# cambrian-mllm/cambrian

Measured on NVIDIA H100. Metric: train_samples_per_sec, higher is better.
Workload: dtype bf16

## Files before the change

cambrian_b200/csrc/attention.cu:

```cuda
#include "common.cuh"
#include <cudaTypedefs.h>
#include <type_traits>

namespace cb {

int make_tmap_bf16_4d(CUtensorMap* out, const void* base, uint64_t d0, uint64_t d1, uint64_t d2, uint64_t d3,
                      uint64_t s1, uint64_t s2, uint64_t s3, uint32_t box_rows);

constexpr float LOG2E = 1.4426950408889634f;

struct AttnParams {
  bf16* o;
  long long o_bs, o_ss;
  float* lse;
  const uint8_t* kmask;
  int B, nh, nkv, Sq, Skv, hd, causal;
  float scale_log2;
};

template <int N>
__device__ __forceinline__ bool keys_all_valid(const uint8_t* km, int k0) {
  constexpr int PER = N / 32;
  static_assert(PER == 2 || PER == 4, "64- or 128-key tiles");
  const uint8_t* kp = km + k0 + PER * (threadIdx.x & 31);
  uint32_t w = 0;
  if (!(reinterpret_cast<uintptr_t>(kp) & (PER - 1))) {
    w = PER == 4 ? *reinterpret_cast<const uint32_t*>(kp) : *reinterpret_cast<const uint16_t*>(kp);
  } else {
#pragma unroll
    for (int i = 0; i < PER; ++i) w |= (uint32_t)kp[i] << (8 * i);
  }
  bool ok = true;
#pragma unroll
  for (int i = 0; i < PER; ++i) ok = ok && ((w >> (8 * i)) & 0xffu);
  return __all_sync(0xffffffffu, ok);
}

struct TileIdx {
  int t, h, b;
};
__device__ __forceinline__ TileIdx tile_index(int heads, int B) {
  const int hb = heads * B;
  const int rem = (int)blockIdx.x % hb;
  return {(int)blockIdx.x / hb, rem % heads, rem / heads};
}

template <int HDP>
struct FwdCfg {
  static constexpr int ATOMS = (HDP + 63) / 64;
  static constexpr int TILE = ATOMS * 16384;
  static constexpr int STAGES = 3;
  static constexpr int SMEM = TILE * (1 + 2 * STAGES) + 1024 + 256;
};

template <int HDP>
__global__ void __launch_bounds__(288, 1)
attn_fwd_kernel(const __grid_constant__ CUtensorMap tmQ, const __grid_constant__ CUtensorMap tmK,
                const __grid_constant__ CUtensorMap tmV, AttnParams p) {
  using Cfg = FwdCfg<HDP>;
  constexpr int STAGES = Cfg::STAGES;
  extern __shared__ uint8_t smem_raw[];
  const uint32_t base = (smem_u32(smem_raw) + 1023u) & ~1023u;
  const uint32_t sQ = base;
  const uint32_t sK = sQ + Cfg::TILE;
  const uint32_t sV = sK + STAGES * Cfg::TILE;
  const uint32_t bars = sV + STAGES * Cfg::TILE;
  const uint32_t q_full = bars;
  auto k_full = [&](int s) { return bars + 8u * (1 + s); };
  auto v_full = [&](int s) { return bars + 8u * (1 + STAGES + s); };
  auto kv_empty = [&](int s) { return bars + 8u * (1 + 2 * STAGES + s); };

  const int warp = threadIdx.x >> 5, lane = threadIdx.x & 31;
  const int q_tiles = (p.Sq + 127) / 128;
  const TileIdx ti = tile_index(p.nh, p.B);
  const int qt = q_tiles - 1 - ti.t;
  const int h = ti.h, b = ti.b;
  const int hk = h / (p.nh / p.nkv);
  const int q0 = qt * 128;
  const int kv_tiles_all = (p.Skv + 127) / 128;
  const int coff = p.Skv - p.Sq;
  int n_tiles = kv_tiles_all;
  if (p.causal) {
    const int last_key = q0 + 127 + coff;
    n_tiles = min(kv_tiles_all, last_key / 128 + 1);
    if (n_tiles < 1) n_tiles = 1;
  }

  if (warp == 8 && lane == 0) {
    tma_prefetch_desc(&tmQ);
    tma_prefetch_desc(&tmK);
    tma_prefetch_desc(&tmV);
    mbar_init(q_full, 1);
    for (int s = 0; s < STAGES; ++s) {
      mbar_init(k_full(s), 1);
      mbar_init(v_full(s), 1);
      mbar_init(kv_empty(s), 2);
    }
    mbar_fence_init();
  }
  __syncthreads();

  if (warp == 8) {
    if (lane == 0) {
      mbar_arrive_expect_tx(q_full, Cfg::TILE);
#pragma unroll
      for (int a = 0; a < Cfg::ATOMS; ++a) tma_load_4d(sQ + a * 16384, &tmQ, q_full, a * 64, h, q0, b);
      int st = 0;
      uint32_t ph = 0;
      for (int j = 0; j < n_tiles; ++j) {
        mbar_wait(kv_empty(st), ph ^ 1u);
        mbar_arrive_expect_tx(k_full(st), Cfg::TILE);
#pragma unroll
        for (int a = 0; a < Cfg::ATOMS; ++a)
          tma_load_4d(sK + st * Cfg::TILE + a * 16384, &tmK, k_full(st), a * 64, hk, j * 128, b);
        mbar_arrive_expect_tx(v_full(st), Cfg::TILE);
#pragma unroll
        for (int a = 0; a < Cfg::ATOMS; ++a)
          tma_load_4d(sV + st * Cfg::TILE + a * 16384, &tmV, v_full(st), a * 64, hk, j * 128, b);
        if (++st == STAGES) { st = 0; ph ^= 1u; }
      }
    }
    return;
  }

  const int wg = warp >> 2;
  const bool wg_leader = (threadIdx.x & 127) == 0;
  const int rloc = wg * 64 + (warp & 3) * 16 + (lane >> 2);
  const int cq = 2 * (lane & 3);
  const uint8_t* km = p.kmask ? p.kmask + (size_t)b * p.Skv : nullptr;
  float o[HDP / 2];
#pragma unroll
  for (int i = 0; i < HDP / 2; ++i) o[i] = 0.f;
  float m_run[2] = {-INFINITY, -INFINITY}, l_run[2] = {0.f, 0.f};
  mbar_wait(q_full, 0);
  int st = 0;
  uint32_t ph = 0;
  for (int j = 0; j < n_tiles; ++j) {
    const int k0 = j * 128;
    float s[64];
    mbar_wait(k_full(st), ph);
    const uint32_t kb = sK + st * Cfg::TILE;
    wgmma_fence();
#pragma unroll
    for (int kk = 0; kk < HDP / 16; ++kk) {
      const uint32_t off = (kk >> 2) * 16384 + (kk & 3) * 32;
      WgmmaSS<128, 0, 0>::mma(s, make_smem_desc_sw128(sQ + wg * 8192 + off, 0, 1024),
                              make_smem_desc_sw128(kb + off, 0, 1024), kk ? 1u : 0u);
    }
    wgmma_commit();
    bool full_tile = k0 + 128 <= p.Skv && (!p.causal || k0 + 127 <= q0 + wg * 64 + coff);
    if (full_tile && km) full_tile = keys_all_valid<128>(km, k0);
    wgmma_wait<0>();
    reg_fence(s);
    float mx[2] = {-INFINITY, -INFINITY};
#pragma unroll
    for (int jj = 0; jj < 16; ++jj) {
#pragma unroll
      for (int e = 0; e < 4; ++e) {
        float v = s[4 * jj + e] * p.scale_log2;
        if (!full_tile) {
          const int key = k0 + 8 * jj + cq + (e & 1);
          const int qi = q0 + rloc + 8 * (e >> 1);
          const bool ok = key < p.Skv && (!p.causal || key <= qi + coff) && (!km || km[key]);
          v = ok ? v : -INFINITY;
        }
        s[4 * jj + e] = v;
        mx[e >> 1] = fmaxf(mx[e >> 1], v);
      }
    }
    float corr[2], mref[2];
#pragma unroll
    for (int r = 0; r < 2; ++r) {
      mx[r] = fmaxf(mx[r], __shfl_xor_sync(0xffffffffu, mx[r], 1));
      mx[r] = fmaxf(mx[r], __shfl_xor_sync(0xffffffffu, mx[r], 2));
      const float m_new = fmaxf(m_run[r], mx[r]);
      mref[r] = m_new == -INFINITY ? 0.f : m_new;
      corr[r] = fast_exp2(m_run[r] - mref[r]);
      m_run[r] = m_new;
      l_run[r] *= corr[r];
    }
#pragma unroll
    for (int jj = 0; jj < HDP / 8; ++jj) {
#pragma unroll
      for (int e = 0; e < 4; ++e) o[4 * jj + e] *= corr[e >> 1];
    }
    uint32_t pa[8][4];
#pragma unroll
    for (int jj = 0; jj < 16; ++jj) {
      float pv[4];
#pragma unroll
      for (int e = 0; e < 4; ++e) {
        pv[e] = fast_exp2(s[4 * jj + e] - mref[e >> 1]);
        l_run[e >> 1] += pv[e];
      }
      pa[jj >> 1][(jj & 1) * 2 + 0] = pack_bf16x2(pv[0], pv[1]);
      pa[jj >> 1][(jj & 1) * 2 + 1] = pack_bf16x2(pv[2], pv[3]);
    }
    mbar_wait(v_full(st), ph);
    const uint32_t vb = sV + st * Cfg::TILE;
    reg_fence(o);
    wgmma_fence();
#pragma unroll
    for (int kk = 0; kk < 8; ++kk)
      WgmmaRS<HDP, 1>::mma(o, pa[kk], make_smem_desc_sw128(vb + kk * 2048, 16384, 1024), 1u);
    wgmma_commit();
    wgmma_wait<0>();
    reg_fence(o);
    if (wg_leader) mbar_arrive(kv_empty(st));
    if (++st == STAGES) { st = 0; ph ^= 1u; }
  }
#pragma unroll
  for (int r = 0; r < 2; ++r) {
    float l = l_run[r];
    l += __shfl_xor_sync(0xffffffffu, l, 1);
    l += __shfl_xor_sync(0xffffffffu, l, 2);
    const int qi = q0 + rloc + 8 * r;
    if (qi >= p.Sq) continue;
    const float inv = l > 0.f ? 1.f / l : 0.f;
    bf16* op = p.o + (long long)b * p.o_bs + (long long)qi * p.o_ss + (long long)h * p.hd;
#pragma unroll
    for (int jj = 0; jj < HDP / 8; ++jj) {
      const int d = 8 * jj + cq;
      if (d < p.hd)
        *reinterpret_cast<__nv_bfloat162*>(op + d) = __floats2bfloat162_rn(o[4 * jj + 2 * r] * inv, o[4 * jj + 2 * r + 1] * inv);
    }
    if (p.lse && (lane & 3) == 0)
      p.lse[((long long)b * p.nh + h) * p.Sq + qi] = l > 0.f ? m_run[r] + log2f(l) : INFINITY;
  }
}

__global__ void attn_delta_kernel(const bf16* __restrict__ o, const bf16* __restrict__ d_o, float* __restrict__ delta,
                                  int B, int S, int nh, int hd, long long o_bs, long long o_ss, long long do_bs,
                                  long long do_ss) {
  const int lph = hd >> 3;
  const int hpw = 32 / lph;
  const long long w = (blockIdx.x * (long long)blockDim.x + threadIdx.x) >> 5;
  const int lane = threadIdx.x & 31;
  const long long total = (long long)B * S * nh;
  const long long idx = w * hpw + lane / lph;
  const int sub = lane % lph;
  float acc = 0.f;
  if (idx < total) {
    const int h = (int)(idx % nh);
    const long long t = idx / nh;
    const int s = (int)(t % S);
    const int b = (int)(t / S);
    const bf16* op = o + b * o_bs + s * o_ss + (long long)h * hd + sub * 8;
    const bf16* gp = d_o + b * do_bs + s * do_ss + (long long)h * hd + sub * 8;
    float a[8], g[8];
    unpack8(ldg_nc(op), a);
    unpack8(ldg_nc(gp), g);
#pragma unroll
    for (int e = 0; e < 8; ++e) acc += a[e] * g[e];
  }
  for (int off = lph >> 1; off > 0; off >>= 1) acc += __shfl_xor_sync(0xffffffffu, acc, off);
  if (idx < total && sub == 0) {
    const int h = (int)(idx % nh);
    const long long t = idx / nh;
    delta[((long long)(t / S) * nh + h) * S + (t % S)] = acc;
  }
}

struct AttnBwdParams {
  bf16* dq;
  bf16* dk;
  bf16* dv;
  long long dq_bs, dq_ss, dk_bs, dk_ss, dv_bs, dv_ss;
  const float* lse;
  const float* delta;
  const uint8_t* kmask;
  int B, nh, nkv, Sq, Skv, hd, causal;
  float scale_log2, scale;
};

template <int HDP>
struct BwdCfg {
  static constexpr int ATOMS = HDP / 64;
  static constexpr int KTILE = ATOMS * 16384;
  static constexpr int QTILE = ATOMS * 8192;
  static constexpr int STAGES = 4;
  static constexpr int SMEM = 2 * KTILE + 2 * STAGES * QTILE + STAGES * 512 + 1024 + 256;
};

template <int HDP>
__global__ void __launch_bounds__(384, 1)
attn_bwd_kernel(const __grid_constant__ CUtensorMap tmQ, const __grid_constant__ CUtensorMap tmK,
                const __grid_constant__ CUtensorMap tmV, const __grid_constant__ CUtensorMap tmdO, AttnBwdParams p) {
  using Cfg = BwdCfg<HDP>;
  constexpr int STAGES = Cfg::STAGES;
  extern __shared__ uint8_t smem_raw[];
  const uint32_t base = (smem_u32(smem_raw) + 1023u) & ~1023u;
  const uint32_t sK = base;
  const uint32_t sV = sK + Cfg::KTILE;
  const uint32_t sQ = sV + Cfg::KTILE;
  const uint32_t sdO = sQ + STAGES * Cfg::QTILE;
  const uint32_t sLD = sdO + STAGES * Cfg::QTILE;
  const uint32_t bars = sLD + STAGES * 512;
  const uint32_t kv_full = bars;
  auto qd_full = [&](int s) { return bars + 8u * (1 + s); };
  auto qd_empty = [&](int s) { return bars + 8u * (1 + STAGES + s); };
  float* ld_stage = reinterpret_cast<float*>(smem_raw + (sLD - smem_u32(smem_raw)));

  const int warp = threadIdx.x >> 5, lane = threadIdx.x & 31;
  const TileIdx ti = tile_index(p.nkv, p.B);
  const int jt = ti.t, g = ti.h, b = ti.b;
  const int G = p.nh / p.nkv;
  const int k0 = jt * 128;
  const int q_tiles = (p.Sq + 63) / 64;
  const int coff = p.Skv - p.Sq;
  int i_begin = 0;
  if (p.causal) {
    const int first_q = k0 - coff;
    i_begin = first_q > 0 ? first_q / 64 : 0;
  }
  const int n_i = q_tiles > i_begin ? q_tiles - i_begin : 0;
  const int n_iter = n_i * G;

  if (warp == 8 && lane == 0) {
    tma_prefetch_desc(&tmQ);
    tma_prefetch_desc(&tmK);
    tma_prefetch_desc(&tmV);
    tma_prefetch_desc(&tmdO);
    mbar_init(kv_full, 1);
    for (int s = 0; s < STAGES; ++s) {
      mbar_init(qd_full(s), 1 + 32);
      mbar_init(qd_empty(s), 8);
    }
    mbar_fence_init();
  }
  __syncthreads();

  if (warp >= 8) {
    setmaxnreg_dec<24>();
    if (warp > 8) return;
    if (lane == 0) {
      mbar_arrive_expect_tx(kv_full, 2 * Cfg::KTILE);
#pragma unroll
      for (int a = 0; a < Cfg::ATOMS; ++a) {
        tma_load_4d(sK + a * 16384, &tmK, kv_full, a * 64, g, k0, b);
        tma_load_4d(sV + a * 16384, &tmV, kv_full, a * 64, g, k0, b);
      }
    }
    int st = 0;
    uint32_t ph = 0;
    for (int it = 0; it < n_iter; ++it) {
      const int h = g * G + it / n_i;
      const int qi0 = (i_begin + it % n_i) * 64;
      mbar_wait(qd_empty(st), ph ^ 1u);
      if (lane == 0) {
        mbar_arrive_expect_tx(qd_full(st), 2 * Cfg::QTILE);
#pragma unroll
        for (int a = 0; a < Cfg::ATOMS; ++a) {
          tma_load_4d(sQ + st * Cfg::QTILE + a * 8192, &tmQ, qd_full(st), a * 64, h, qi0, b);
          tma_load_4d(sdO + st * Cfg::QTILE + a * 8192, &tmdO, qd_full(st), a * 64, h, qi0, b);
        }
      }
      const float* lse = p.lse + ((long long)b * p.nh + h) * p.Sq;
      const float* dlt = p.delta + ((long long)b * p.nh + h) * p.Sq;
      float* ld = ld_stage + st * 128;
#pragma unroll
      for (int i = lane; i < 64; i += 32) {
        const int qi = qi0 + i;
        ld[i] = qi < p.Sq ? __ldg(lse + qi) : 0.f;
        ld[64 + i] = qi < p.Sq ? __ldg(dlt + qi) : 0.f;
      }
      mbar_arrive(qd_full(st));
      if (++st == STAGES) { st = 0; ph ^= 1u; }
    }
    return;
  }

  setmaxnreg_inc<240>();
  const int wg = warp >> 2;
  const int kr = wg * 64 + (warp & 3) * 16 + (lane >> 2);
  const int cq = 2 * (lane & 3);
  const int wk0 = k0 + wg * 64 + (warp & 3) * 16;
  bool key_ok[2];
#pragma unroll
  for (int r = 0; r < 2; ++r) {
    const int kidx = k0 + kr + 8 * r;
    key_ok[r] = kidx < p.Skv && (!p.kmask || p.kmask[(size_t)b * p.Skv + kidx]);
  }
  const bool warp_keys_ok = __all_sync(0xffffffffu, key_ok[0] && key_ok[1]);
  float dv[HDP / 2], dk[HDP / 2];
#pragma unroll
  for (int i = 0; i < HDP / 2; ++i) dv[i] = dk[i] = 0.f;
  mbar_wait(kv_full, 0);
  int st = 0;
  uint32_t ph = 0;
  for (int it = 0; it < n_iter; ++it) {
    const int qi0 = (i_begin + it % n_i) * 64;
    const uint32_t qb = sQ + st * Cfg::QTILE, dob = sdO + st * Cfg::QTILE;
    mbar_wait(qd_full(st), ph);
    float sT[32], dpT[32];
    wgmma_fence();
#pragma unroll
    for (int kk = 0; kk < HDP / 16; ++kk) {
      const uint32_t koff = (kk >> 2) * 16384 + (kk & 3) * 32, qoff = (kk >> 2) * 8192 + (kk & 3) * 32;
      WgmmaSS<64, 0, 0>::mma(sT, make_smem_desc_sw128(sK + wg * 8192 + koff, 0, 1024),
                             make_smem_desc_sw128(qb + qoff, 0, 1024), kk ? 1u : 0u);
    }
#pragma unroll
    for (int kk = 0; kk < HDP / 16; ++kk) {
      const uint32_t koff = (kk >> 2) * 16384 + (kk & 3) * 32, qoff = (kk >> 2) * 8192 + (kk & 3) * 32;
      WgmmaSS<64, 0, 0>::mma(dpT, make_smem_desc_sw128(sV + wg * 8192 + koff, 0, 1024),
                             make_smem_desc_sw128(dob + qoff, 0, 1024), kk ? 1u : 0u);
    }
    wgmma_commit();
    const bool full = warp_keys_ok && qi0 + 64 <= p.Sq && (!p.causal || wk0 + 15 <= qi0 + coff);
    const float* ld = ld_stage + st * 128;
    wgmma_wait<0>();
    reg_fence(sT);
    reg_fence(dpT);
    uint32_t pa[4][4], da[4][4];
    auto grads = [&](auto full_tile) {
#pragma unroll
      for (int jj = 0; jj < 8; ++jj) {
        float pv[4], dsv[4];
#pragma unroll
        for (int c = 0; c < 2; ++c) {
          const int qc = 8 * jj + cq + c;
          const float L = ld[qc], D = ld[64 + qc];
#pragma unroll
          for (int r = 0; r < 2; ++r) {
            const int e = 2 * r + c;
            bool vis = true;
            if (!decltype(full_tile)::value)
              vis = qi0 + qc < p.Sq && key_ok[r] && (!p.causal || k0 + kr + 8 * r <= qi0 + qc + coff);
            const float pe = vis ? fast_exp2(fmaf(sT[4 * jj + e], p.scale_log2, -L)) : 0.f;
            pv[e] = pe;
            dsv[e] = pe * (dpT[4 * jj + e] - D);
          }
        }
        pa[jj >> 1][(jj & 1) * 2 + 0] = pack_bf16x2(pv[0], pv[1]);
        pa[jj >> 1][(jj & 1) * 2 + 1] = pack_bf16x2(pv[2], pv[3]);
        da[jj >> 1][(jj & 1) * 2 + 0] = pack_bf16x2(dsv[0], dsv[1]);
        da[jj >> 1][(jj & 1) * 2 + 1] = pack_bf16x2(dsv[2], dsv[3]);
      }
    };
    if (full)
      grads(std::true_type());
    else
      grads(std::false_type());
    reg_fence(dv);
    reg_fence(dk);
    wgmma_fence();
#pragma unroll
    for (int kk = 0; kk < 4; ++kk) {
      WgmmaRS<HDP, 1>::mma(dv, pa[kk], make_smem_desc_sw128(dob + kk * 2048, 8192, 1024), 1u);
      WgmmaRS<HDP, 1>::mma(dk, da[kk], make_smem_desc_sw128(qb + kk * 2048, 8192, 1024), 1u);
    }
    wgmma_commit();
    wgmma_wait<0>();
    reg_fence(dv);
    reg_fence(dk);
    if (lane == 0) mbar_arrive(qd_empty(st));
    if (++st == STAGES) { st = 0; ph ^= 1u; }
  }
#pragma unroll
  for (int r = 0; r < 2; ++r) {
    const int kidx = k0 + kr + 8 * r;
    if (kidx >= p.Skv) continue;
    bf16* dkp = p.dk + (long long)b * p.dk_bs + (long long)kidx * p.dk_ss + (long long)g * p.hd;
    bf16* dvp = p.dv + (long long)b * p.dv_bs + (long long)kidx * p.dv_ss + (long long)g * p.hd;
#pragma unroll
    for (int jj = 0; jj < HDP / 8; ++jj) {
      const int d = 8 * jj + cq;
      *reinterpret_cast<__nv_bfloat162*>(dkp + d) =
          __floats2bfloat162_rn(dk[4 * jj + 2 * r] * p.scale, dk[4 * jj + 2 * r + 1] * p.scale);
      *reinterpret_cast<__nv_bfloat162*>(dvp + d) = __floats2bfloat162_rn(dv[4 * jj + 2 * r], dv[4 * jj + 2 * r + 1]);
    }
  }
}

template <int HDP>
struct DqCfg {
  static constexpr int ATOMS = HDP / 64;
  static constexpr int QTILE = ATOMS * 16384;
  static constexpr int KTILE = ATOMS * 8192;
  static constexpr int STAGES = 4;
  static constexpr int SMEM = 2 * QTILE + 2 * STAGES * KTILE + 1024 + 256;
};

template <int HDP>
__global__ void __launch_bounds__(288, 1)
attn_bwd_dq_kernel(const __grid_constant__ CUtensorMap tmQ, const __grid_constant__ CUtensorMap tmK,
                   const __grid_constant__ CUtensorMap tmV, const __grid_constant__ CUtensorMap tmdO, AttnBwdParams p) {
  using Cfg = DqCfg<HDP>;
  constexpr int STAGES = Cfg::STAGES;
  extern __shared__ uint8_t smem_raw[];
  const uint32_t base = (smem_u32(smem_raw) + 1023u) & ~1023u;
  const uint32_t sQ = base;
  const uint32_t sdO = sQ + Cfg::QTILE;
  const uint32_t sK = sdO + Cfg::QTILE;
  const uint32_t sV = sK + STAGES * Cfg::KTILE;
  const uint32_t bars = sV + STAGES * Cfg::KTILE;
  const uint32_t q_full = bars;
  auto kv_full = [&](int s) { return bars + 8u * (1 + s); };
  auto kv_empty = [&](int s) { return bars + 8u * (1 + STAGES + s); };

  const int warp = threadIdx.x >> 5, lane = threadIdx.x & 31;
  const int q_tiles = (p.Sq + 127) / 128;
  const TileIdx ti = tile_index(p.nh, p.B);
  const int qt = q_tiles - 1 - ti.t;
  const int h = ti.h, b = ti.b;
  const int hk = h / (p.nh / p.nkv);
  const int q0 = qt * 128;
  const int coff = p.Skv - p.Sq;
  const int kv_tiles_all = (p.Skv + 63) / 64;
  int n_tiles = kv_tiles_all;
  if (p.causal) n_tiles = max(1, min(kv_tiles_all, (q0 + 127 + coff) / 64 + 1));

  if (warp == 8 && lane == 0) {
    tma_prefetch_desc(&tmQ);
    tma_prefetch_desc(&tmK);
    tma_prefetch_desc(&tmV);
    tma_prefetch_desc(&tmdO);
    mbar_init(q_full, 1);
    for (int s = 0; s < STAGES; ++s) {
      mbar_init(kv_full(s), 1);
      mbar_init(kv_empty(s), 2);
    }
    mbar_fence_init();
  }
  __syncthreads();

  if (warp == 8) {
    if (lane == 0) {
      mbar_arrive_expect_tx(q_full, 2 * Cfg::QTILE);
#pragma unroll
      for (int a = 0; a < Cfg::ATOMS; ++a) {
        tma_load_4d(sQ + a * 16384, &tmQ, q_full, a * 64, h, q0, b);
        tma_load_4d(sdO + a * 16384, &tmdO, q_full, a * 64, h, q0, b);
      }
      int st = 0;
      uint32_t ph = 0;
      for (int j = 0; j < n_tiles; ++j) {
        mbar_wait(kv_empty(st), ph ^ 1u);
        mbar_arrive_expect_tx(kv_full(st), 2 * Cfg::KTILE);
#pragma unroll
        for (int a = 0; a < Cfg::ATOMS; ++a) {
          tma_load_4d(sK + st * Cfg::KTILE + a * 8192, &tmK, kv_full(st), a * 64, hk, j * 64, b);
          tma_load_4d(sV + st * Cfg::KTILE + a * 8192, &tmV, kv_full(st), a * 64, hk, j * 64, b);
        }
        if (++st == STAGES) { st = 0; ph ^= 1u; }
      }
    }
    return;
  }

  const int wg = warp >> 2;
  const bool wg_leader = (threadIdx.x & 127) == 0;
  const int rloc = wg * 64 + (warp & 3) * 16 + (lane >> 2);
  const int cq = 2 * (lane & 3);
  const int wq0 = q0 + wg * 64 + (warp & 3) * 16;
  const uint8_t* km = p.kmask ? p.kmask + (size_t)b * p.Skv : nullptr;
  const float* lse = p.lse + ((long long)b * p.nh + h) * p.Sq;
  const float* dlt = p.delta + ((long long)b * p.nh + h) * p.Sq;
  int qi[2];
  float L[2], D[2];
#pragma unroll
  for (int r = 0; r < 2; ++r) {
    qi[r] = q0 + rloc + 8 * r;
    L[r] = qi[r] < p.Sq ? __ldg(lse + qi[r]) : 0.f;
    D[r] = qi[r] < p.Sq ? __ldg(dlt + qi[r]) : 0.f;
  }
  float dq[HDP / 2];
#pragma unroll
  for (int i = 0; i < HDP / 2; ++i) dq[i] = 0.f;
  mbar_wait(q_full, 0);
  int st = 0;
  uint32_t ph = 0;
  for (int j = 0; j < n_tiles; ++j) {
    const int k0 = j * 64;
    mbar_wait(kv_full(st), ph);
    const uint32_t kb = sK + st * Cfg::KTILE, vb = sV + st * Cfg::KTILE;
    float s[32], dp[32];
    wgmma_fence();
#pragma unroll
    for (int kk = 0; kk < HDP / 16; ++kk) {
      const uint32_t qoff = wg * 8192 + (kk >> 2) * 16384 + (kk & 3) * 32, koff = (kk >> 2) * 8192 + (kk & 3) * 32;
      WgmmaSS<64, 0, 0>::mma(s, make_smem_desc_sw128(sQ + qoff, 0, 1024), make_smem_desc_sw128(kb + koff, 0, 1024),
                             kk ? 1u : 0u);
    }
#pragma unroll
    for (int kk = 0; kk < HDP / 16; ++kk) {
      const uint32_t qoff = wg * 8192 + (kk >> 2) * 16384 + (kk & 3) * 32, koff = (kk >> 2) * 8192 + (kk & 3) * 32;
      WgmmaSS<64, 0, 0>::mma(dp, make_smem_desc_sw128(sdO + qoff, 0, 1024), make_smem_desc_sw128(vb + koff, 0, 1024),
                             kk ? 1u : 0u);
    }
    wgmma_commit();
    bool full = k0 + 64 <= p.Skv && wq0 + 16 <= p.Sq && (!p.causal || k0 + 63 <= wq0 + coff);
    if (full && km) full = keys_all_valid<64>(km, k0);
    wgmma_wait<0>();
    reg_fence(s);
    reg_fence(dp);
    uint32_t da[4][4];
    auto grads = [&](auto full_tile) {
#pragma unroll
      for (int jj = 0; jj < 8; ++jj) {
        float dsv[4];
#pragma unroll
        for (int e = 0; e < 4; ++e) {
          const int r = e >> 1, key = k0 + 8 * jj + cq + (e & 1);
          bool vis = true;
          if (!decltype(full_tile)::value)
            vis = qi[r] < p.Sq && key < p.Skv && (!p.causal || key <= qi[r] + coff) && (!km || km[key]);
          const float pe = vis ? fast_exp2(fmaf(s[4 * jj + e], p.scale_log2, -L[r])) : 0.f;
          dsv[e] = pe * (dp[4 * jj + e] - D[r]);
        }
        da[jj >> 1][(jj & 1) * 2 + 0] = pack_bf16x2(dsv[0], dsv[1]);
        da[jj >> 1][(jj & 1) * 2 + 1] = pack_bf16x2(dsv[2], dsv[3]);
      }
    };
    if (full)
      grads(std::true_type());
    else
      grads(std::false_type());
    reg_fence(dq);
    wgmma_fence();
#pragma unroll
    for (int kk = 0; kk < 4; ++kk)
      WgmmaRS<HDP, 1>::mma(dq, da[kk], make_smem_desc_sw128(kb + kk * 2048, 8192, 1024), 1u);
    wgmma_commit();
    wgmma_wait<0>();
    reg_fence(dq);
    if (wg_leader) mbar_arrive(kv_empty(st));
    if (++st == STAGES) { st = 0; ph ^= 1u; }
  }
#pragma unroll
  for (int r = 0; r < 2; ++r) {
    if (qi[r] >= p.Sq) continue;
    bf16* dqp = p.dq + (long long)b * p.dq_bs + (long long)qi[r] * p.dq_ss + (long long)h * p.hd;
#pragma unroll
    for (int jj = 0; jj < HDP / 8; ++jj)
      *reinterpret_cast<__nv_bfloat162*>(dqp + 8 * jj + cq) =
          __floats2bfloat162_rn(dq[4 * jj + 2 * r] * p.scale, dq[4 * jj + 2 * r + 1] * p.scale);
  }
}

static PFN_cuTensorMapEncodeTiled_v12000 encode_fn() {
  static PFN_cuTensorMapEncodeTiled_v12000 fn = nullptr;
  if (!fn) {
    void* ptr = nullptr;
    cudaDriverEntryPointQueryResult q;
    if (cudaGetDriverEntryPoint("cuTensorMapEncodeTiled", &ptr, cudaEnableDefault, &q) == cudaSuccess &&
        q == cudaDriverEntryPointSuccess)
      fn = reinterpret_cast<PFN_cuTensorMapEncodeTiled_v12000>(ptr);
  }
  return fn;
}

int make_tmap_bf16_4d(CUtensorMap* out, const void* base, uint64_t d0, uint64_t d1, uint64_t d2, uint64_t d3,
                      uint64_t s1, uint64_t s2, uint64_t s3, uint32_t box_rows) {
  auto fn = encode_fn();
  if (!fn) return set_error(CB_ERR_CUDA, "cuTensorMapEncodeTiled entry point not available");
  if ((reinterpret_cast<uintptr_t>(base) & 15u) || (s1 % 8) || (s2 % 8) || (d3 > 1 && (s3 % 8)))
    return set_error(CB_ERR_INVALID, "attention: operands must be 16-byte aligned with strides %% 8 == 0");
  cuuint64_t dims[4] = {d0, d1, d2, d3};
  cuuint64_t strides[3] = {s1 * 2, s2 * 2, (d3 > 1 ? s3 : s2 * d2) * 2};
  cuuint32_t box[4] = {64, 1, box_rows, 1};
  cuuint32_t estr[4] = {1, 1, 1, 1};
  CUresult r = fn(out, CU_TENSOR_MAP_DATA_TYPE_BFLOAT16, 4, const_cast<void*>(base), dims, strides, box, estr,
                  CU_TENSOR_MAP_INTERLEAVE_NONE, CU_TENSOR_MAP_SWIZZLE_128B, CU_TENSOR_MAP_L2_PROMOTION_L2_256B,
                  CU_TENSOR_MAP_FLOAT_OOB_FILL_NONE);
  if (r == CUDA_ERROR_INVALID_CONTEXT) {
    cudaFree(0);
    r = fn(out, CU_TENSOR_MAP_DATA_TYPE_BFLOAT16, 4, const_cast<void*>(base), dims, strides, box, estr,
           CU_TENSOR_MAP_INTERLEAVE_NONE, CU_TENSOR_MAP_SWIZZLE_128B, CU_TENSOR_MAP_L2_PROMOTION_L2_256B,
           CU_TENSOR_MAP_FLOAT_OOB_FILL_NONE);
  }
  if (r != CUDA_SUCCESS) return set_error(CB_ERR_CUDA, "cuTensorMapEncodeTiled(4d) failed (%d)", (int)r);
  return CB_OK;
}

static int hd_padded(int hd) { return (hd + 15) / 16 * 16; }

template <int HDP>
static int launch_fwd(const CUtensorMap& tq, const CUtensorMap& tk, const CUtensorMap& tv, const AttnParams& p,
                      cudaStream_t st) {
  using Cfg = FwdCfg<HDP>;
  auto kern = attn_fwd_kernel<HDP>;
  static bool attr = false;
  if (!attr) {
    cudaError_t e = cudaFuncSetAttribute(kern, cudaFuncAttributeMaxDynamicSharedMemorySize, Cfg::SMEM);
    if (e != cudaSuccess) return set_error(CB_ERR_CUDA, "attn fwd smem attr: %s", cudaGetErrorString(e));
    attr = true;
  }
  kern<<<(p.Sq + 127) / 128 * p.nh * p.B, 288, Cfg::SMEM, st>>>(tq, tk, tv, p);
  CB_CUDA_LAUNCH_CHECK("attn_fwd");
  return CB_OK;
}

int attn_fwd_launch(const void* q, const void* k, const void* v, void* o, float* lse, const void* kmask, int B,
                    int nh, int nkv, int Sq, int Skv, int hd, long long q_bs, long long q_ss, long long k_bs,
                    long long k_ss, long long v_bs, long long v_ss, long long o_bs, long long o_ss, float scale,
                    int causal, cudaStream_t st) {
  CB_CHECK_ARG(B > 0 && nh > 0 && nkv > 0 && Sq > 0 && Skv > 0, "attention: empty problem");
  CB_CHECK_ARG(nh % nkv == 0, "attention: nh=%d not a multiple of nkv=%d", nh, nkv);
  CB_CHECK_ARG(hd % 8 == 0 && hd <= 128, "attention: head_dim=%d must be a multiple of 8 and <= 128", hd);
  CB_CHECK_ARG(o_ss % 8 == 0 && o_bs % 8 == 0 && !(reinterpret_cast<uintptr_t>(o) & 15u),
               "attention: output must be 16-byte aligned with strides %% 8 == 0");
  CUtensorMap tq, tk, tv;
  int rc;
  if ((rc = make_tmap_bf16_4d(&tq, q, hd, nh, Sq, B, hd, q_ss, q_bs, 128))) return rc;
  if ((rc = make_tmap_bf16_4d(&tk, k, hd, nkv, Skv, B, hd, k_ss, k_bs, 128))) return rc;
  if ((rc = make_tmap_bf16_4d(&tv, v, hd, nkv, Skv, B, hd, v_ss, v_bs, 128))) return rc;
  AttnParams p;
  p.o = (bf16*)o; p.o_bs = o_bs; p.o_ss = o_ss; p.lse = lse; p.kmask = (const uint8_t*)kmask;
  p.B = B; p.nh = nh; p.nkv = nkv; p.Sq = Sq; p.Skv = Skv; p.hd = hd; p.causal = causal;
  p.scale_log2 = scale * LOG2E;
  const int hdp = hd_padded(hd);
  if (hdp <= 64) return launch_fwd<64>(tq, tk, tv, p, st);
  if (hdp <= 80) return launch_fwd<80>(tq, tk, tv, p, st);
  if (hdp <= 96) return launch_fwd<96>(tq, tk, tv, p, st);
  return launch_fwd<128>(tq, tk, tv, p, st);
}

template <int HDP>
static int launch_bwd(const CUtensorMap& tq, const CUtensorMap& tk, const CUtensorMap& tv, const CUtensorMap& tdo,
                      const AttnBwdParams& p, cudaStream_t st) {
  using Cfg = BwdCfg<HDP>;
  auto kern = attn_bwd_kernel<HDP>;
  static bool attr = false;
  if (!attr) {
    cudaError_t e = cudaFuncSetAttribute(kern, cudaFuncAttributeMaxDynamicSharedMemorySize, Cfg::SMEM);
    if (e != cudaSuccess) return set_error(CB_ERR_CUDA, "attn bwd smem attr: %s", cudaGetErrorString(e));
    attr = true;
  }
  kern<<<(p.Skv + 127) / 128 * p.nkv * p.B, 384, Cfg::SMEM, st>>>(tq, tk, tv, tdo, p);
  CB_CUDA_LAUNCH_CHECK("attn_bwd");
  return CB_OK;
}

template <int HDP>
static int launch_bwd_dq(const CUtensorMap& tq, const CUtensorMap& tk, const CUtensorMap& tv, const CUtensorMap& tdo,
                         const AttnBwdParams& p, cudaStream_t st) {
  using Cfg = DqCfg<HDP>;
  auto kern = attn_bwd_dq_kernel<HDP>;
  static bool attr = false;
  if (!attr) {
    cudaError_t e = cudaFuncSetAttribute(kern, cudaFuncAttributeMaxDynamicSharedMemorySize, Cfg::SMEM);
    if (e != cudaSuccess) return set_error(CB_ERR_CUDA, "attn bwd dq smem attr: %s", cudaGetErrorString(e));
    attr = true;
  }
  kern<<<(p.Sq + 127) / 128 * p.nh * p.B, 288, Cfg::SMEM, st>>>(tq, tk, tv, tdo, p);
  CB_CUDA_LAUNCH_CHECK("attn_bwd_dq");
  return CB_OK;
}

int attn_bwd_launch(const void* q, const void* k, const void* v, const void* o, const void* d_o, const float* lse,
                    float* delta, void* dq, void* dk, void* dv, const void* kmask, int B, int nh, int nkv,
                    int Sq, int Skv, int hd, long long q_bs, long long q_ss, long long k_bs, long long k_ss,
                    long long v_bs, long long v_ss, long long o_bs, long long o_ss, long long do_bs, long long do_ss,
                    long long dq_bs, long long dq_ss, long long dk_bs, long long dk_ss, long long dv_bs,
                    long long dv_ss, float scale, int causal, cudaStream_t st) {
  CB_CHECK_ARG(B > 0 && nh > 0 && nkv > 0 && Sq > 0 && Skv > 0, "attention bwd: empty problem");
  CB_CHECK_ARG(nh % nkv == 0, "attention bwd: nh=%d not a multiple of nkv=%d", nh, nkv);
  CB_CHECK_ARG(hd == 64 || hd == 128, "attention bwd: head_dim=%d unsupported (64 or 128)", hd);
  CB_CHECK_ARG(lse && delta && dq && dk && dv, "attention bwd: lse / delta / dq / dk / dv buffers are required");
  CB_CHECK_ARG(!(reinterpret_cast<uintptr_t>(dq) & 3u) && dq_bs % 2 == 0 && dq_ss % 2 == 0,
               "attention bwd: dq must be 4-byte aligned with even strides");
  {
    const long long warps = ((long long)B * Sq * nh + (256 / hd) - 1) / (256 / hd);
    attn_delta_kernel<<<(unsigned)((warps * 32 + 255) / 256), 256, 0, st>>>((const bf16*)o, (const bf16*)d_o, delta, B,
                                                                           Sq, nh, hd, o_bs, o_ss, do_bs, do_ss);
    CB_CUDA_LAUNCH_CHECK("attn_delta");
  }
  CUtensorMap tq, tk, tv, tdo;
  int rc;
  if ((rc = make_tmap_bf16_4d(&tq, q, hd, nh, Sq, B, hd, q_ss, q_bs, 64))) return rc;
  if ((rc = make_tmap_bf16_4d(&tk, k, hd, nkv, Skv, B, hd, k_ss, k_bs, 128))) return rc;
  if ((rc = make_tmap_bf16_4d(&tv, v, hd, nkv, Skv, B, hd, v_ss, v_bs, 128))) return rc;
  if ((rc = make_tmap_bf16_4d(&tdo, d_o, hd, nh, Sq, B, hd, do_ss, do_bs, 64))) return rc;
  AttnBwdParams p;
  p.dq = (bf16*)dq; p.dk = (bf16*)dk; p.dv = (bf16*)dv;
  p.dq_bs = dq_bs; p.dq_ss = dq_ss; p.dk_bs = dk_bs; p.dk_ss = dk_ss; p.dv_bs = dv_bs; p.dv_ss = dv_ss;
  p.lse = lse; p.delta = delta; p.kmask = (const uint8_t*)kmask;
  p.B = B; p.nh = nh; p.nkv = nkv; p.Sq = Sq; p.Skv = Skv; p.hd = hd; p.causal = causal;
  p.scale_log2 = scale * LOG2E; p.scale = scale;
  CUtensorMap tq128, tk64, tv64, tdo128;
  if ((rc = make_tmap_bf16_4d(&tq128, q, hd, nh, Sq, B, hd, q_ss, q_bs, 128))) return rc;
  if ((rc = make_tmap_bf16_4d(&tk64, k, hd, nkv, Skv, B, hd, k_ss, k_bs, 64))) return rc;
  if ((rc = make_tmap_bf16_4d(&tv64, v, hd, nkv, Skv, B, hd, v_ss, v_bs, 64))) return rc;
  if ((rc = make_tmap_bf16_4d(&tdo128, d_o, hd, nh, Sq, B, hd, do_ss, do_bs, 128))) return rc;
  if (hd == 64) {
    if ((rc = launch_bwd<64>(tq, tk, tv, tdo, p, st))) return rc;
    return launch_bwd_dq<64>(tq128, tk64, tv64, tdo128, p, st);
  }
  if ((rc = launch_bwd<128>(tq, tk, tv, tdo, p, st))) return rc;
  return launch_bwd_dq<128>(tq128, tk64, tv64, tdo128, p, st);
}

}
```

cambrian_b200/csrc/common.cuh:

```cuda
#pragma once
#include <cuda_runtime.h>
#include <cuda_bf16.h>
#include <cuda.h>
#include <stdint.h>
#include "wgmma.cuh"

namespace cb {

typedef __nv_bfloat16 bf16;

int set_error(int code, const char* fmt, ...);
#define CB_OK 0
#define CB_ERR_INVALID 1
#define CB_ERR_CUDA 2
#define CB_ERR_UNSUPPORTED 3

#define CB_CHECK_ARG(cond, ...)                                         \
  do {                                                                  \
    if (!(cond)) return cb::set_error(CB_ERR_INVALID, __VA_ARGS__);     \
  } while (0)

void count_launch();
#define CB_CUDA_LAUNCH_CHECK(name)                                                    \
  do {                                                                                \
    cb::count_launch();                                                               \
    cudaError_t _e = cudaGetLastError();                                              \
    if (_e != cudaSuccess)                                                            \
      return cb::set_error(CB_ERR_CUDA, "%s: %s", name, cudaGetErrorString(_e));      \
  } while (0)

int device_sm_count();

__device__ __forceinline__ float warp_sum(float v) {
#pragma unroll
  for (int o = 16; o > 0; o >>= 1) v += __shfl_xor_sync(0xffffffffu, v, o);
  return v;
}
__device__ __forceinline__ float warp_max(float v) {
#pragma unroll
  for (int o = 16; o > 0; o >>= 1) v = fmaxf(v, __shfl_xor_sync(0xffffffffu, v, o));
  return v;
}

__device__ __forceinline__ float fast_exp2(float x) {
  float y;
  asm("ex2.approx.ftz.f32 %0, %1;" : "=f"(y) : "f"(x));
  return y;
}
__device__ __forceinline__ float fast_rcp(float x) {
  float y;
  asm("rcp.approx.ftz.f32 %0, %1;" : "=f"(y) : "f"(x));
  return y;
}
__device__ __forceinline__ float erf_fast(float x) {
  const float ax = fabsf(x);
  const float t = __fdividef(1.0f, fmaf(0.3275911f, ax, 1.0f));
  float y = fmaf(t, 1.061405429f, -1.453152027f);
  y = fmaf(t, y, 1.421413741f);
  y = fmaf(t, y, -0.284496736f);
  y = fmaf(t, y, 0.254829592f);
  const float r = fmaf(-t * y, __expf(-ax * ax), 1.0f);
  return copysignf(r, x);
}
__device__ __forceinline__ float gelu_erf(float x) {
  const float ax = fabsf(x);
  const float t = fast_rcp(fmaf(0.3275911f * 0.70710678118654752440f, ax, 1.0f));
  float y = fmaf(t, 1.061405429f, -1.453152027f);
  y = fmaf(t, y, 1.421413741f);
  y = fmaf(t, y, -0.284496736f);
  y = fmaf(t, y, 0.254829592f);
  const float e = fast_exp2(x * x * -0.72134752044448170368f);
  const float r = fmaf(-(y * t), e, 1.0f);
  const float hx = 0.5f * x;
  return fmaf(fabsf(hx), r, hx);
}
__device__ __forceinline__ float gelu_erf_grad(float x) {
  const float cdf = 0.5f * (1.0f + erf_fast(x * 0.70710678118654752440f));
  const float pdf = 0.39894228040143267794f * __expf(-0.5f * x * x);
  return cdf + x * pdf;
}
__device__ __forceinline__ float gelu_tanh(float x) {
  const float u = 0.7978845608028654f * (x + 0.044715f * x * x * x);
  return 0.5f * x * (1.0f + tanhf(u));
}
__device__ __forceinline__ float gelu_tanh_fast(float x) {
  const float u = 0.7978845608028654f * (x + 0.044715f * x * x * x);
  const float t = 1.0f - 2.0f * fast_rcp(1.0f + fast_exp2(2.0f * 1.44269504088896340736f * u));
  return 0.5f * x * (1.0f + t);
}
__device__ __forceinline__ float quick_gelu(float x) { return x * fast_rcp(1.0f + fast_exp2(-1.702f * 1.44269504088896340736f * x)); }
__device__ __forceinline__ float silu(float x) { return x * fast_rcp(1.0f + fast_exp2(-1.44269504088896340736f * x)); }

struct alignas(16) bf16x8 {
  __nv_bfloat162 v[4];
};
__device__ __forceinline__ void unpack8(const uint4& u, float* f) {
  const __nv_bfloat162* p = reinterpret_cast<const __nv_bfloat162*>(&u);
#pragma unroll
  for (int i = 0; i < 4; ++i) {
    float2 t = __bfloat1622float2(p[i]);
    f[2 * i] = t.x;
    f[2 * i + 1] = t.y;
  }
}
__device__ __forceinline__ uint4 pack8(const float* f) {
  uint4 u;
  __nv_bfloat162* p = reinterpret_cast<__nv_bfloat162*>(&u);
#pragma unroll
  for (int i = 0; i < 4; ++i) p[i] = __floats2bfloat162_rn(f[2 * i], f[2 * i + 1]);
  return u;
}
__device__ __forceinline__ uint4 ldg_nc(const void* p) {
  uint4 r;
  asm volatile("ld.global.nc.L1::no_allocate.v4.u32 {%0,%1,%2,%3}, [%4];"
               : "=r"(r.x), "=r"(r.y), "=r"(r.z), "=r"(r.w)
               : "l"(p));
  return r;
}

__device__ __forceinline__ uint32_t smem_u32(const void* p) {
  return static_cast<uint32_t>(__cvta_generic_to_shared(p));
}
__device__ __forceinline__ void mbar_init(uint32_t bar, uint32_t count) {
  asm volatile("mbarrier.init.shared::cta.b64 [%0], %1;" ::"r"(bar), "r"(count));
}
__device__ __forceinline__ void mbar_fence_init() {
  asm volatile("fence.mbarrier_init.release.cluster;" ::: "memory");
}
__device__ __forceinline__ void mbar_arrive_expect_tx(uint32_t bar, uint32_t bytes) {
  asm volatile("mbarrier.arrive.expect_tx.shared::cta.b64 _, [%0], %1;" ::"r"(bar), "r"(bytes)
               : "memory");
}
__device__ __forceinline__ void mbar_arrive(uint32_t bar) {
  asm volatile("mbarrier.arrive.shared::cta.b64 _, [%0];" ::"r"(bar) : "memory");
}
__device__ __forceinline__ void mbar_wait(uint32_t bar, uint32_t parity) {
  uint32_t done;
  do {
    asm volatile(
        "{\n"
        ".reg .pred p;\n"
        "mbarrier.try_wait.parity.shared::cta.b64 p, [%1], %2;\n"
        "selp.u32 %0, 1, 0, p;\n"
        "}\n"
        : "=r"(done)
        : "r"(bar), "r"(parity)
        : "memory");
  } while (!done);
}
__device__ __forceinline__ void st_shared_b32(uint32_t addr, uint32_t v) {
  asm volatile("st.shared.b32 [%0], %1;" ::"r"(addr), "r"(v) : "memory");
}
__device__ __forceinline__ void fence_proxy_async_smem() {
  asm volatile("fence.proxy.async.shared::cta;" ::: "memory");
}

__device__ __forceinline__ void tma_prefetch_desc(const CUtensorMap* m) {
  asm volatile("prefetch.tensormap [%0];" ::"l"(m) : "memory");
}
__device__ __forceinline__ void tma_load_3d(uint32_t smem_dst, const CUtensorMap* m, uint32_t bar,
                                            int c0, int c1, int c2) {
  asm volatile(
      "cp.async.bulk.tensor.3d.shared::cluster.global.mbarrier::complete_tx::bytes "
      "[%0], [%1, {%3, %4, %5}], [%2];"
      :
      : "r"(smem_dst), "l"(m), "r"(bar), "r"(c0), "r"(c1), "r"(c2)
      : "memory");
}
__device__ __forceinline__ void tma_load_4d(uint32_t smem_dst, const CUtensorMap* m, uint32_t bar,
                                            int c0, int c1, int c2, int c3) {
  asm volatile(
      "cp.async.bulk.tensor.4d.shared::cluster.global.mbarrier::complete_tx::bytes "
      "[%0], [%1, {%3, %4, %5, %6}], [%2];"
      :
      : "r"(smem_dst), "l"(m), "r"(bar), "r"(c0), "r"(c1), "r"(c2), "r"(c3)
      : "memory");
}
__device__ __forceinline__ void tma_store_3d(const CUtensorMap* m, uint32_t smem_src, int c0, int c1, int c2) {
  asm volatile("cp.async.bulk.tensor.3d.global.shared::cta.bulk_group [%0, {%2, %3, %4}], [%1];"
               :
               : "l"(m), "r"(smem_src), "r"(c0), "r"(c1), "r"(c2)
               : "memory");
}
__device__ __forceinline__ void bulk_commit() { asm volatile("cp.async.bulk.commit_group;" ::: "memory"); }
template <int N>
__device__ __forceinline__ void bulk_wait_read() {
  asm volatile("cp.async.bulk.wait_group.read %0;" ::"n"(N) : "memory");
}
template <int N>
__device__ __forceinline__ void bulk_wait() {
  asm volatile("cp.async.bulk.wait_group %0;" ::"n"(N) : "memory");
}
template <int N>
__device__ __forceinline__ void setmaxnreg_dec() { asm volatile("setmaxnreg.dec.sync.aligned.u32 %0;" ::"n"(N)); }
template <int N>
__device__ __forceinline__ void setmaxnreg_inc() { asm volatile("setmaxnreg.inc.sync.aligned.u32 %0;" ::"n"(N)); }
__device__ __forceinline__ void named_bar_sync(int id, int threads) {
  asm volatile("bar.sync %0, %1;" ::"r"(id), "r"(threads) : "memory");
}

__device__ __forceinline__ void wgmma_fence() { asm volatile("wgmma.fence.sync.aligned;" ::: "memory"); }
__device__ __forceinline__ void wgmma_commit() { asm volatile("wgmma.commit_group.sync.aligned;" ::: "memory"); }
template <int N>
__device__ __forceinline__ void wgmma_wait() {
  asm volatile("wgmma.wait_group.sync.aligned %0;" ::"n"(N) : "memory");
}
template <int R>
__device__ __forceinline__ void reg_fence(float (&d)[R]) {
#pragma unroll
  for (int i = 0; i < R; ++i) asm volatile("" : "+f"(d[i])::"memory");
}

__device__ __forceinline__ uint64_t make_smem_desc_sw128(uint32_t saddr, uint32_t lbo_bytes,
                                                         uint32_t sbo_bytes) {
  uint64_t d = 0;
  d |= static_cast<uint64_t>((saddr & 0x3FFFFu) >> 4);
  d |= static_cast<uint64_t>((lbo_bytes >> 4) & 0x3FFFu) << 16;
  d |= static_cast<uint64_t>((sbo_bytes >> 4) & 0x3FFFu) << 32;
  d |= static_cast<uint64_t>(1) << 62;
  return d;
}

__device__ __forceinline__ uint32_t pack_bf16x2(float lo, float hi) {
  __nv_bfloat162 t = __floats2bfloat162_rn(lo, hi);
  return *reinterpret_cast<uint32_t*>(&t);
}

}
```

Before: 7.913.

## Make attention fwd/bwd-dq kernels persistent with pingpong warpgroups and TMA output stores

Converts the attention forward and backward-dQ kernels into persistent kernels that loop over work tiles in serpentine order, launching at most one CTA per SM. A double-buffered Q stage is added, and K and V get separate empty barriers. The two consumer warpgroups are interleaved with named barriers (pingpong), and the next S GEMM is overlapped with the current PV GEMM. Register budgets are reallocated with setmaxnreg, and the output is written through a TMA store from shared memory when alignment allows. This targets launch and tail overhead and aims to hide softmax latency behind tensor-core work, at the cost of much more complex synchronisation and fewer pipeline stages.

```diff
diff --git a/cambrian_b200/csrc/attention.cu b/cambrian_b200/csrc/attention.cu
--- a/cambrian_b200/csrc/attention.cu
+++ b/cambrian_b200/csrc/attention.cu
@@ -1,5 +1,6 @@
 #include "common.cuh"
 #include <cudaTypedefs.h>
+#include <algorithm>
 #include <type_traits>
 
 namespace cb {
@@ -16,6 +17,7 @@
   const uint8_t* kmask;
   int B, nh, nkv, Sq, Skv, hd, causal;
   float scale_log2;
+  int tma_store;
 };
 
 template <int N>
@@ -39,194 +41,298 @@
 struct TileIdx {
   int t, h, b;
 };
-__device__ __forceinline__ TileIdx tile_index(int heads, int B) {
+__device__ __forceinline__ TileIdx tile_index(int w, int heads, int B) {
   const int hb = heads * B;
-  const int rem = (int)blockIdx.x % hb;
-  return {(int)blockIdx.x / hb, rem % heads, rem / heads};
+  const int rem = w % hb;
+  return {w / hb, rem % heads, rem / heads};
+}
+__device__ __forceinline__ int work_tile(int k) {
+  const int G = gridDim.x, c = blockIdx.x;
+  return k * G + ((k & 1) ? G - 1 - c : c);
 }
 
 template <int HDP>
 struct FwdCfg {
   static constexpr int ATOMS = (HDP + 63) / 64;
   static constexpr int TILE = ATOMS * 16384;
-  static constexpr int STAGES = 3;
-  static constexpr int SMEM = TILE * (1 + 2 * STAGES) + 1024 + 256;
+  static constexpr int SMEM = 6 * TILE + 1024 + 256;
 };
 
 template <int HDP>
-__global__ void __launch_bounds__(288, 1)
+__global__ void __launch_bounds__(384, 1)
 attn_fwd_kernel(const __grid_constant__ CUtensorMap tmQ, const __grid_constant__ CUtensorMap tmK,
-                const __grid_constant__ CUtensorMap tmV, AttnParams p) {
+                const __grid_constant__ CUtensorMap tmV, const __grid_constant__ CUtensorMap tmO, AttnParams p) {
   using Cfg = FwdCfg<HDP>;
-  constexpr int STAGES = Cfg::STAGES;
   extern __shared__ uint8_t smem_raw[];
   const uint32_t base = (smem_u32(smem_raw) + 1023u) & ~1023u;
   const uint32_t sQ = base;
-  const uint32_t sK = sQ + Cfg::TILE;
-  const uint32_t sV = sK + STAGES * Cfg::TILE;
-  const uint32_t bars = sV + STAGES * Cfg::TILE;
-  const uint32_t q_full = bars;
-  auto k_full = [&](int s) { return bars + 8u * (1 + s); };
-  auto v_full = [&](int s) { return bars + 8u * (1 + STAGES + s); };
-  auto kv_empty = [&](int s) { return bars + 8u * (1 + 2 * STAGES + s); };
+  const uint32_t sK = sQ + 2 * Cfg::TILE;
+  const uint32_t sV = sK + 2 * Cfg::TILE;
+  const uint32_t bars = sV + 2 * Cfg::TILE;
+  auto q_full = [&](int s) { return bars + 8u * s; };
+  auto q_empty = [&](int s) { return bars + 8u * (2 + s); };
+  auto k_full = [&](int s) { return bars + 8u * (4 + s); };
+  auto k_empty = [&](int s) { return bars + 8u * (6 + s); };
+  auto v_full = [&](int s) { return bars + 8u * (8 + s); };
+  auto v_empty = [&](int s) { return bars + 8u * (10 + s); };
 
   const int warp = threadIdx.x >> 5, lane = threadIdx.x & 31;
   const int q_tiles = (p.Sq + 127) / 128;
-  const TileIdx ti = tile_index(p.nh, p.B);
-  const int qt = q_tiles - 1 - ti.t;
-  const int h = ti.h, b = ti.b;
-  const int hk = h / (p.nh / p.nkv);
-  const int q0 = qt * 128;
+  const int work = q_tiles * p.nh * p.B;
   const int kv_tiles_all = (p.Skv + 127) / 128;
   const int coff = p.Skv - p.Sq;
-  int n_tiles = kv_tiles_all;
-  if (p.causal) {
-    const int last_key = q0 + 127 + coff;
-    n_tiles = min(kv_tiles_all, last_key / 128 + 1);
-    if (n_tiles < 1) n_tiles = 1;
-  }
+  auto key_tiles = [&](int q0) {
+    return p.causal ? max(1, min(kv_tiles_all, (q0 + 127 + coff) / 128 + 1)) : kv_tiles_all;
+  };
 
   if (warp == 8 && lane == 0) {
     tma_prefetch_desc(&tmQ);
     tma_prefetch_desc(&tmK);
     tma_prefetch_desc(&tmV);
-    mbar_init(q_full, 1);
-    for (int s = 0; s < STAGES; ++s) {
+    for (int s = 0; s < 2; ++s) {
+      mbar_init(q_full(s), 1);
+      mbar_init(q_empty(s), 2);
       mbar_init(k_full(s), 1);
+      mbar_init(k_empty(s), 2);
       mbar_init(v_full(s), 1);
-      mbar_init(kv_empty(s), 2);
+      mbar_init(v_empty(s), 2);
     }
     mbar_fence_init();
   }
   __syncthreads();
 
-  if (warp == 8) {
-    if (lane == 0) {
-      mbar_arrive_expect_tx(q_full, Cfg::TILE);
-#pragma unroll
-      for (int a = 0; a < Cfg::ATOMS; ++a) tma_load_4d(sQ + a * 16384, &tmQ, q_full, a * 64, h, q0, b);
-      int st = 0;
-      uint32_t ph = 0;
-      for (int j = 0; j < n_tiles; ++j) {
-        mbar_wait(kv_empty(st), ph ^ 1u);
-        mbar_arrive_expect_tx(k_full(st), Cfg::TILE);
+  if (warp >= 8) {
+    setmaxnreg_dec<24>();
+    if (warp == 8 && lane == 0) {
+      int qs = 0, st = 0;
+      uint32_t qph = 0, ph = 0;
+      for (int k = 0, w; (w = work_tile(k)) < work; ++k) {
+        const TileIdx ti = tile_index(w, p.nh, p.B);
+        const int q0 = (q_tiles - 1 - ti.t) * 128;
+        const int hk = ti.h / (p.nh / p.nkv);
+        mbar_wait(q_empty(qs), qph ^ 1u);
+        mbar_arrive_expect_tx(q_full(qs), Cfg::TILE);
 #pragma unroll
         for (int a = 0; a < Cfg::ATOMS; ++a)
-          tma_load_4d(sK + st * Cfg::TILE + a * 16384, &tmK, k_full(st), a * 64, hk, j * 128, b);
-        mbar_arrive_expect_tx(v_full(st), Cfg::TILE);
-#pragma unroll
-        for (int a = 0; a < Cfg::ATOMS; ++a)
-          tma_load_4d(sV + st * Cfg::TILE + a * 16384, &tmV, v_full(st), a * 64, hk, j * 128, b);
-        if (++st == STAGES) { st = 0; ph ^= 1u; }
+          tma_load_4d(sQ + qs * Cfg::TILE + a * 16384, &tmQ, q_full(qs), a * 64, ti.h, q0, ti.b);
+        if (++qs == 2) { qs = 0; qph ^= 1u; }
+        const int n_tiles = key_tiles(q0);
+        for (int j = 0; j < n_tiles; ++j) {
+          mbar_wait(k_empty(st), ph ^ 1u);
+          mbar_arrive_expect_tx(k_full(st), Cfg::TILE);
+#pragma unroll
+          for (int a = 0; a < Cfg::ATOMS; ++a)
+            tma_load_4d(sK + st * Cfg::TILE + a * 16384, &tmK, k_full(st), a * 64, hk, j * 128, ti.b);
+          mbar_wait(v_empty(st), ph ^ 1u);
+          mbar_arrive_expect_tx(v_full(st), Cfg::TILE);
+#pragma unroll
+          for (int a = 0; a < Cfg::ATOMS; ++a)
+            tma_load_4d(sV + st * Cfg::TILE + a * 16384, &tmV, v_full(st), a * 64, hk, j * 128, ti.b);
+          if (++st == 2) { st = 0; ph ^= 1u; }
+        }
       }
     }
     return;
   }
 
+  setmaxnreg_inc<240>();
   const int wg = warp >> 2;
   const bool wg_leader = (threadIdx.x & 127) == 0;
-  const int rloc = wg * 64 + (warp & 3) * 16 + (lane >> 2);
+  const int srow = (warp & 3) * 16 + (lane >> 2);
+  const int rloc = wg * 64 + srow;
   const int cq = 2 * (lane & 3);
-  const uint8_t* km = p.kmask ? p.kmask + (size_t)b * p.Skv : nullptr;
-  float o[HDP / 2];
-#pragma unroll
-  for (int i = 0; i < HDP / 2; ++i) o[i] = 0.f;
-  float m_run[2] = {-INFINITY, -INFINITY}, l_run[2] = {0.f, 0.f};
-  mbar_wait(q_full, 0);
-  int st = 0;
-  uint32_t ph = 0;
-  for (int j = 0; j < n_tiles; ++j) {
-    const int k0 = j * 128;
-    float s[64];
-    mbar_wait(k_full(st), ph);
-    const uint32_t kb = sK + st * Cfg::TILE;
+  const int bar_mine = 1 + wg, bar_other = 2 - wg;
+  if (wg == 1) named_bar_arrive(1, 256);
+  if (wg_leader && p.tma_store) tma_prefetch_desc(&tmO);
+
+  int qs = 0, kst = 0, vst = 0;
+  uint32_t qph = 0, kph = 0, vph = 0;
+  int q_release = -1;
+  for (int k = 0, w; (w = work_tile(k)) < work; ++k) {
+    const TileIdx ti = tile_index(w, p.nh, p.B);
+    const int q0 = (q_tiles - 1 - ti.t) * 128;
+    const int h = ti.h, b = ti.b;
+    const int n_tiles = key_tiles(q0);
+    const uint8_t* km = p.kmask ? p.kmask + (size_t)b * p.Skv : nullptr;
+    const uint32_t qb = sQ + qs * Cfg::TILE + wg * 8192;
+    float o[HDP / 2], s[64];
+    uint32_t pa[8][4];
+#pragma unroll
+    for (int i = 0; i < HDP / 2; ++i) o[i] = 0.f;
+    float m_run[2] = {-INFINITY, -INFINITY}, l_run[2] = {0.f, 0.f}, corr[2];
+
+    auto issue_s = [&]() {
+      const uint32_t kb = sK + kst * Cfg::TILE;
+#pragma unroll
+      for (int kk = 0; kk < HDP / 16; ++kk) {
+        const uint32_t off = (kk >> 2) * 16384 + (kk & 3) * 32;
+        WgmmaSS<128, 0, 0>::mma(s, make_smem_desc_sw128(qb + off, 0, 1024), make_smem_desc_sw128(kb + off, 0, 1024),
+                                kk ? 1u : 0u);
+      }
+      wgmma_commit();
+    };
+    auto tile_full = [&](int k0) {
+      bool full = k0 + 128 <= p.Skv && (!p.causal || k0 + 127 <= q0 + wg * 64 + coff);
+      if (full && km) full = keys_all_valid<128>(km, k0);
+      return full;
+    };
+    auto softmax = [&](int k0, bool full_tile) {
+      float mx[2] = {-INFINITY, -INFINITY};
+#pragma unroll
+      for (int jj = 0; jj < 16; ++jj) {
+#pragma unroll
+        for (int e = 0; e < 4; ++e) {
+          float v = s[4 * jj + e] * p.scale_log2;
+          if (!full_tile) {
+            const int key = k0 + 8 * jj + cq + (e & 1);
+            const int qi = q0 + rloc + 8 * (e >> 1);
+            const bool ok = key < p.Skv && (!p.causal || key <= qi + coff) && (!km || km[key]);
+            v = ok ? v : -INFINITY;
+          }
+          s[4 * jj + e] = v;
+          mx[e >> 1] = fmaxf(mx[e >> 1], v);
+        }
+      }
+      float mref[2];
+#pragma unroll
+      for (int r = 0; r < 2; ++r) {
+        mx[r] = fmaxf(mx[r], __shfl_xor_sync(0xffffffffu, mx[r], 1));
+        mx[r] = fmaxf(mx[r], __shfl_xor_sync(0xffffffffu, mx[r], 2));
+        const float m_new = fmaxf(m_run[r], mx[r]);
+        mref[r] = m_new == -INFINITY ? 0.f : m_new;
+        corr[r] = fast_exp2(m_run[r] - mref[r]);
+        m_run[r] = m_new;
+        l_run[r] *= corr[r];
+      }
+#pragma unroll
+      for (int jj = 0; jj < 16; ++jj) {
+#pragma unroll
+        for (int e = 0; e < 4; ++e) {
+          s[4 * jj + e] = fast_exp2(s[4 * jj + e] - mref[e >> 1]);
+          l_run[e >> 1] += s[4 * jj + e];
+        }
+      }
+    };
+    auto rescale_pack = [&]() {
+#pragma unroll
+      for (int jj = 0; jj < HDP / 8; ++jj) {
+#pragma unroll
+        for (int e = 0; e < 4; ++e) o[4 * jj + e] *= corr[e >> 1];
+      }
+#pragma unroll
+      for (int jj = 0; jj < 16; ++jj) {
+        pa[jj >> 1][(jj & 1) * 2 + 0] = pack_bf16x2(s[4 * jj + 0], s[4 * jj + 1]);
+        pa[jj >> 1][(jj & 1) * 2 + 1] = pack_bf16x2(s[4 * jj + 2], s[4 * jj + 3]);
+      }
+    };
+
+    mbar_wait(q_full(qs), qph);
+    mbar_wait(k_full(kst), kph);
+    named_bar_sync(bar_mine, 256);
     wgmma_fence();
-#pragma unroll
-    for (int kk = 0; kk < HDP / 16; ++kk) {
-      const uint32_t off = (kk >> 2) * 16384 + (kk & 3) * 32;
-      WgmmaSS<128, 0, 0>::mma(s, make_smem_desc_sw128(sQ + wg * 8192 + off, 0, 1024),
-                              make_smem_desc_sw128(kb + off, 0, 1024), kk ? 1u : 0u);
-    }
-    wgmma_commit();
-    bool full_tile = k0 + 128 <= p.Skv && (!p.causal || k0 + 127 <= q0 + wg * 64 + coff);
-    if (full_tile && km) full_tile = keys_all_valid<128>(km, k0);
-    wgmma_wait<0>();
-    reg_fence(s);
-    float mx[2] = {-INFINITY, -INFINITY};
-#pragma unroll
-    for (int jj = 0; jj < 16; ++jj) {
-#pragma unroll
-      for (int e = 0; e < 4; ++e) {
-        float v = s[4 * jj + e] * p.scale_log2;
-        if (!full_tile) {
-          const int key = k0 + 8 * jj + cq + (e & 1);
-          const int qi = q0 + rloc + 8 * (e >> 1);
-          const bool ok = key < p.Skv && (!p.causal || key <= qi + coff) && (!km || km[key]);
-          v = ok ? v : -INFINITY;
-        }
-        s[4 * jj + e] = v;
-        mx[e >> 1] = fmaxf(mx[e >> 1], v);
-      }
-    }
-    float corr[2], mref[2];
-#pragma unroll
-    for (int r = 0; r < 2; ++r) {
-      mx[r] = fmaxf(mx[r], __shfl_xor_sync(0xffffffffu, mx[r], 1));
-      mx[r] = fmaxf(mx[r], __shfl_xor_sync(0xffffffffu, mx[r], 2));
-      const float m_new = fmaxf(m_run[r], mx[r]);
-      mref[r] = m_new == -INFINITY ? 0.f : m_new;
-      corr[r] = fast_exp2(m_run[r] - mref[r]);
-      m_run[r] = m_new;
-      l_run[r] *= corr[r];
-    }
-#pragma unroll
-    for (int jj = 0; jj < HDP / 8; ++jj) {
-#pragma unroll
-      for (int e = 0; e < 4; ++e) o[4 * jj + e] *= corr[e >> 1];
-    }
-    uint32_t pa[8][4];
-#pragma unroll
-    for (int jj = 0; jj < 16; ++jj) {
-      float pv[4];
-#pragma unroll
-      for (int e = 0; e < 4; ++e) {
-        pv[e] = fast_exp2(s[4 * jj + e] - mref[e >> 1]);
-        l_run[e >> 1] += pv[e];
-      }
-      pa[jj >> 1][(jj & 1) * 2 + 0] = pack_bf16x2(pv[0], pv[1]);
-      pa[jj >> 1][(jj & 1) * 2 + 1] = pack_bf16x2(pv[2], pv[3]);
-    }
-    mbar_wait(v_full(st), ph);
-    const uint32_t vb = sV + st * Cfg::TILE;
+    issue_s();
+    named_bar_arrive(bar_other, 256);
+    if (q_release >= 0 && wg_leader) {
+      if (p.tma_store) bulk_wait_read<0>();
+      mbar_arrive(q_empty(q_release));
+    }
+    {
+      const bool full = tile_full(0);
+      wgmma_wait<0>();
+      reg_fence(s);
+      if (wg_leader) mbar_arrive(k_empty(kst));
+      if (++kst == 2) { kst = 0; kph ^= 1u; }
+      softmax(0, full);
+      rescale_pack();
+    }
+    auto issue_pv = [&]() {
+      const uint32_t vb = sV + vst * Cfg::TILE;
+#pragma unroll
+      for (int kk = 0; kk < 8; ++kk)
+        WgmmaRS<HDP, 1>::mma(o, pa[kk], make_smem_desc_sw128(vb + kk * 2048, 16384, 1024), 1u);
+      wgmma_commit();
+    };
+    auto release_v = [&]() {
+      if (wg_leader) mbar_arrive(v_empty(vst));
+      if (++vst == 2) { vst = 0; vph ^= 1u; }
+    };
+    for (int j = 0; j + 1 < n_tiles; ++j) {
+      mbar_wait(k_full(kst), kph);
+      mbar_wait(v_full(vst), vph);
+      named_bar_sync(bar_mine, 256);
+      reg_fence(o);
+      wgmma_fence();
+      issue_s();
+      issue_pv();
+      named_bar_arrive(bar_other, 256);
+      const int k1 = (j + 1) * 128;
+      const bool full = tile_full(k1);
+      wgmma_wait<1>();
+      reg_fence(s);
+      if (wg_leader) mbar_arrive(k_empty(kst));
+      if (++kst == 2) { kst = 0; kph ^= 1u; }
+      softmax(k1, full);
+      wgmma_wait<0>();
+      reg_fence(o);
+      release_v();
+      rescale_pack();
+    }
+    mbar_wait(v_full(vst), vph);
+    named_bar_sync(bar_mine, 256);
     reg_fence(o);
     wgmma_fence();
-#pragma unroll
-    for (int kk = 0; kk < 8; ++kk)
-      WgmmaRS<HDP, 1>::mma(o, pa[kk], make_smem_desc_sw128(vb + kk * 2048, 16384, 1024), 1u);
-    wgmma_commit();
+    issue_pv();
+    named_bar_arrive(bar_other, 256);
     wgmma_wait<0>();
     reg_fence(o);
-    if (wg_leader) mbar_arrive(kv_empty(st));
-    if (++st == STAGES) { st = 0; ph ^= 1u; }
-  }
-#pragma unroll
-  for (int r = 0; r < 2; ++r) {
-    float l = l_run[r];
-    l += __shfl_xor_sync(0xffffffffu, l, 1);
-    l += __shfl_xor_sync(0xffffffffu, l, 2);
-    const int qi = q0 + rloc + 8 * r;
-    if (qi >= p.Sq) continue;
-    const float inv = l > 0.f ? 1.f / l : 0.f;
-    bf16* op = p.o + (long long)b * p.o_bs + (long long)qi * p.o_ss + (long long)h * p.hd;
-#pragma unroll
-    for (int jj = 0; jj < HDP / 8; ++jj) {
-      const int d = 8 * jj + cq;
-      if (d < p.hd)
-        *reinterpret_cast<__nv_bfloat162*>(op + d) = __floats2bfloat162_rn(o[4 * jj + 2 * r] * inv, o[4 * jj + 2 * r + 1] * inv);
-    }
-    if (p.lse && (lane & 3) == 0)
-      p.lse[((long long)b * p.nh + h) * p.Sq + qi] = l > 0.f ? m_run[r] + log2f(l) : INFINITY;
-  }
+    release_v();
+    float inv[2];
+#pragma unroll
+    for (int r = 0; r < 2; ++r) {
+      float l = l_run[r];
+      l += __shfl_xor_sync(0xffffffffu, l, 1);
+      l += __shfl_xor_sync(0xffffffffu, l, 2);
+      inv[r] = l > 0.f ? 1.f / l : 0.f;
+      const int qi = q0 + rloc + 8 * r;
+      if (p.lse && (lane & 3) == 0 && qi < p.Sq)
+        p.lse[((long long)b * p.nh + h) * p.Sq + qi] = l > 0.f ? m_run[r] + log2f(l) : INFINITY;
+    }
+    if (p.tma_store) {
+#pragma unroll
+      for (int r = 0; r < 2; ++r) {
+        const int row = srow + 8 * r;
+#pragma unroll
+        for (int jj = 0; jj < HDP / 8; ++jj)
+          st_shared_b32(qb + (jj >> 3) * 16384 + row * 128 + (((jj & 7) ^ (row & 7)) << 4) + 2 * cq,
+                        pack_bf16x2(o[4 * jj + 2 * r] * inv[r], o[4 * jj + 2 * r + 1] * inv[r]));
+      }
+      fence_proxy_async_smem();
+      named_bar_sync(3 + wg, 128);
+      if (wg_leader) {
+#pragma unroll
+        for (int a = 0; a < Cfg::ATOMS; ++a) tma_store_4d(&tmO, qb + a * 16384, a * 64, h, q0 + wg * 64, b);
+        bulk_commit();
+      }
+    } else {
+#pragma unroll
+      for (int r = 0; r < 2; ++r) {
+        const int qi = q0 + rloc + 8 * r;
+        if (qi >= p.Sq) continue;
+        bf16* op = p.o + (long long)b * p.o_bs + (long long)qi * p.o_ss + (long long)h * p.hd;
+#pragma unroll
+        for (int jj = 0; jj < HDP / 8; ++jj) {
+          const int d = 8 * jj + cq;
+          if (d < p.hd)
+            *reinterpret_cast<__nv_bfloat162*>(op + d) =
+                __floats2bfloat162_rn(o[4 * jj + 2 * r] * inv[r], o[4 * jj + 2 * r + 1] * inv[r]);
+        }
+      }
+    }
+    q_release = qs;
+    if (++qs == 2) { qs = 0; qph ^= 1u; }
+  }
+  if (wg == 0) named_bar_sync(1, 256);
+  if (wg_leader && p.tma_store) bulk_wait<0>();
 }
 
 __global__ void attn_delta_kernel(const bf16* __restrict__ o, const bf16* __restrict__ d_o, float* __restrict__ delta,
@@ -302,7 +408,7 @@
   float* ld_stage = reinterpret_cast<float*>(smem_raw + (sLD - smem_u32(smem_raw)));
 
   const int warp = threadIdx.x >> 5, lane = threadIdx.x & 31;
-  const TileIdx ti = tile_index(p.nkv, p.B);
+  const TileIdx ti = tile_index(blockIdx.x, p.nkv, p.B);
   const int jt = ti.t, g = ti.h, b = ti.b;
   const int G = p.nh / p.nkv;
   const int k0 = jt * 128;
@@ -478,12 +584,12 @@
   static constexpr int ATOMS = HDP / 64;
   static constexpr int QTILE = ATOMS * 16384;
   static constexpr int KTILE = ATOMS * 8192;
-  static constexpr int STAGES = 4;
-  static constexpr int SMEM = 2 * QTILE + 2 * STAGES * KTILE + 1024 + 256;
+  static constexpr int STAGES = 3;
+  static constexpr int SMEM = 4 * QTILE + 2 * STAGES * KTILE + 1024 + 256;
 };
 
 template <int HDP>
-__global__ void __launch_bounds__(288, 1)
+__global__ void __launch_bounds__(384, 1)
 attn_bwd_dq_kernel(const __grid_constant__ CUtensorMap tmQ, const __grid_constant__ CUtensorMap tmK,
                    const __grid_constant__ CUtensorMap tmV, const __grid_constant__ CUtensorMap tmdO, AttnBwdParams p) {
   using Cfg = DqCfg<HDP>;
@@ -491,32 +597,33 @@
   extern __shared__ uint8_t smem_raw[];
   const uint32_t base = (smem_u32(smem_raw) + 1023u) & ~1023u;
   const uint32_t sQ = base;
-  const uint32_t sdO = sQ + Cfg::QTILE;
-  const uint32_t sK = sdO + Cfg::QTILE;
+  const uint32_t sdO = sQ + 2 * Cfg::QTILE;
+  const uint32_t sK = sdO + 2 * Cfg::QTILE;
   const uint32_t sV = sK + STAGES * Cfg::KTILE;
   const uint32_t bars = sV + STAGES * Cfg::KTILE;
-  const uint32_t q_full = bars;
-  auto kv_full = [&](int s) { return bars + 8u * (1 + s); };
-  auto kv_empty = [&](int s) { return bars + 8u * (1 + STAGES + s); };
+  auto q_full = [&](int s) { return bars + 8u * s; };
+  auto q_empty = [&](int s) { return bars + 8u * (2 + s); };
+  auto kv_full = [&](int s) { return bars + 8u * (4 + s); };
+  auto kv_empty = [&](int s) { return bars + 8u * (4 + STAGES + s); };
 
   const int warp = threadIdx.x >> 5, lane = threadIdx.x & 31;
   const int q_tiles = (p.Sq + 127) / 128;
-  const TileIdx ti = tile_index(p.nh, p.B);
-  const int qt = q_tiles - 1 - ti.t;
-  const int h = ti.h, b = ti.b;
-  const int hk = h / (p.nh / p.nkv);
-  const int q0 = qt * 128;
+  const int work = q_tiles * p.nh * p.B;
   const int coff = p.Skv - p.Sq;
   const int kv_tiles_all = (p.Skv + 63) / 64;
-  int n_tiles = kv_tiles_all;
-  if (p.causal) n_tiles = max(1, min(kv_tiles_all, (q0 + 127 + coff) / 64 + 1));
+  auto key_tiles = [&](int q0) {
+    return p.causal ? max(1, min(kv_tiles_all, (q0 + 127 + coff) / 64 + 1)) : kv_tiles_all;
+  };
 
   if (warp == 8 && lane == 0) {
     tma_prefetch_desc(&tmQ);
     tma_prefetch_desc(&tmK);
     tma_prefetch_desc(&tmV);
     tma_prefetch_desc(&tmdO);
-    mbar_init(q_full, 1);
+    for (int s = 0; s < 2; ++s) {
+      mbar_init(q_full(s), 1);
+      mbar_init(q_empty(s), 2);
+    }
     for (int s = 0; s < STAGES; ++s) {
       mbar_init(kv_full(s), 1);
       mbar_init(kv_empty(s), 2);
@@ -525,81 +632,108 @@
   }
   __syncthreads();
 
-  if (warp == 8) {
-    if (lane == 0) {
-      mbar_arrive_expect_tx(q_full, 2 * Cfg::QTILE);
-#pragma unroll
-      for (int a = 0; a < Cfg::ATOMS; ++a) {
-        tma_load_4d(sQ + a * 16384, &tmQ, q_full, a * 64, h, q0, b);
-        tma_load_4d(sdO + a * 16384, &tmdO, q_full, a * 64, h, q0, b);
-      }
-      int st = 0;
-      uint32_t ph = 0;
-      for (int j = 0; j < n_tiles; ++j) {
-        mbar_wait(kv_empty(st), ph ^ 1u);
-        mbar_arrive_expect_tx(kv_full(st), 2 * Cfg::KTILE);
+  if (warp >= 8) {
+    setmaxnreg_dec<24>();
+    if (warp == 8 && lane == 0) {
+      int qs = 0, st = 0;
+      uint32_t qph = 0, ph = 0;
+      for (int k = 0, w; (w = work_tile(k)) < work; ++k) {
+        const TileIdx ti = tile_index(w, p.nh, p.B);
+        const int q0 = (q_tiles - 1 - ti.t) * 128;
+        const int hk = ti.h / (p.nh / p.nkv);
+        mbar_wait(q_empty(qs), qph ^ 1u);
+        mbar_arrive_expect_tx(q_full(qs), 2 * Cfg::QTILE);
 #pragma unroll
         for (int a = 0; a < Cfg::ATOMS; ++a) {
-          tma_load_4d(sK + st * Cfg::KTILE + a * 8192, &tmK, kv_full(st), a * 64, hk, j * 64, b);
-          tma_load_4d(sV + st * Cfg::KTILE + a * 8192, &tmV, kv_full(st), a * 64, hk, j * 64, b);
+          tma_load_4d(sQ + qs * Cfg::QTILE + a * 16384, &tmQ, q_full(qs), a * 64, ti.h, q0, ti.b);
+          tma_load_4d(sdO + qs * Cfg::QTILE + a * 16384, &tmdO, q_full(qs), a * 64, ti.h, q0, ti.b);
         }
-        if (++st == STAGES) { st = 0; ph ^= 1u; }
+        if (++qs == 2) { qs = 0; qph ^= 1u; }
+        const int n_tiles = key_tiles(q0);
+        for (int j = 0; j < n_tiles; ++j) {
+          mbar_wait(kv_empty(st), ph ^ 1u);
+          mbar_arrive_expect_tx(kv_full(st), 2 * Cfg::KTILE);
+#pragma unroll
+          for (int a = 0; a < Cfg::ATOMS; ++a) {
+            tma_load_4d(sK + st * Cfg::KTILE + a * 8192, &tmK, kv_full(st), a * 64, hk, j * 64, ti.b);
+            tma_load_4d(sV + st * Cfg::KTILE + a * 8192, &tmV, kv_full(st), a * 64, hk, j * 64, ti.b);
+          }
+          if (++st == STAGES) { st = 0; ph ^= 1u; }
+        }
       }
     }
     return;
   }
 
+  setmaxnreg_inc<240>();
   const int wg = warp >> 2;
   const bool wg_leader = (threadIdx.x & 127) == 0;
   const int rloc = wg * 64 + (warp & 3) * 16 + (lane >> 2);
   const int cq = 2 * (lane & 3);
-  const int wq0 = q0 + wg * 64 + (warp & 3) * 16;
-  const uint8_t* km = p.kmask ? p.kmask + (size_t)b * p.Skv : nullptr;
-  const float* lse = p.lse + ((long long)b * p.nh + h) * p.Sq;
-  const float* dlt = p.delta + ((long long)b * p.nh + h) * p.Sq;
-  int qi[2];
-  float L[2], D[2];
-#pragma unroll
-  for (int r = 0; r < 2; ++r) {
-    qi[r] = q0 + rloc + 8 * r;
-    L[r] = qi[r] < p.Sq ? __ldg(lse + qi[r]) : 0.f;
-    D[r] = qi[r] < p.Sq ? __ldg(dlt + qi[r]) : 0.f;
-  }
-  float dq[HDP / 2];
-#pragma unroll
-  for (int i = 0; i < HDP / 2; ++i) dq[i] = 0.f;
-  mbar_wait(q_full, 0);
-  int st = 0;
-  uint32_t ph = 0;
-  for (int j = 0; j < n_tiles; ++j) {
-    const int k0 = j * 64;
-    mbar_wait(kv_full(st), ph);
-    const uint32_t kb = sK + st * Cfg::KTILE, vb = sV + st * Cfg::KTILE;
-    float s[32], dp[32];
-    wgmma_fence();
-#pragma unroll
-    for (int kk = 0; kk < HDP / 16; ++kk) {
-      const uint32_t qoff = wg * 8192 + (kk >> 2) * 16384 + (kk & 3) * 32, koff = (kk >> 2) * 8192 + (kk & 3) * 32;
-      WgmmaSS<64, 0, 0>::mma(s, make_smem_desc_sw128(sQ + qoff, 0, 1024), make_smem_desc_sw128(kb + koff, 0, 1024),
-                             kk ? 1u : 0u);
-    }
-#pragma unroll
-    for (int kk = 0; kk < HDP / 16; ++kk) {
-      const uint32_t qoff = wg * 8192 + (kk >> 2) * 16384 + (kk & 3) * 32, koff = (kk >> 2) * 8192 + (kk & 3) * 32;
-      WgmmaSS<64, 0, 0>::mma(dp, make_smem_desc_sw128(sdO + qoff, 0, 1024), make_smem_desc_sw128(vb + koff, 0, 1024),
-                             kk ? 1u : 0u);
-    }
-    wgmma_commit();
-    bool full = k0 + 64 <= p.Skv && wq0 + 16 <= p.Sq && (!p.causal || k0 + 63 <= wq0 + coff);
-    if (full && km) full = keys_all_valid<64>(km, k0);
-    wgmma_wait<0>();
-    reg_fence(s);
-    reg_fence(dp);
+  const int bar_mine = 1 + wg, bar_other = 2 - wg;
+  if (wg == 1) named_bar_arrive(1, 256);
+
+  int qs = 0, ist = 0, rst = 0;
+  uint32_t qph = 0, iph = 0;
+  for (int k = 0, w; (w = work_tile(k)) < work; ++k) {
+    const TileIdx ti = tile_index(w, p.nh, p.B);
+    const int q0 = (q_tiles - 1 - ti.t) * 128;
+    const int h = ti.h, b = ti.b;
+    const int n_tiles = key_tiles(q0);
+    const int wq0 = q0 + wg * 64 + (warp & 3) * 16;
+    const uint8_t* km = p.kmask ? p.kmask + (size_t)b * p.Skv : nullptr;
+    const float* lse = p.lse + ((long long)b * p.nh + h) * p.Sq;
+    const float* dlt = p.delta + ((long long)b * p.nh + h) * p.Sq;
+    int qi[2];
+    float L[2], D[2];
+#pragma unroll
+    for (int r = 0; r < 2; ++r) {
+      qi[r] = q0 + rloc + 8 * r;
+      L[r] = qi[r] < p.Sq ? __ldg(lse + qi[r]) : 0.f;
+      D[r] = qi[r] < p.Sq ? __ldg(dlt + qi[r]) : 0.f;
+    }
+    const uint32_t qb = sQ + qs * Cfg::QTILE + wg * 8192, dob = sdO + qs * Cfg::QTILE + wg * 8192;
+    float dq[HDP / 2], s[32], dp[32];
     uint32_t da[4][4];
-    auto grads = [&](auto full_tile) {
+#pragma unroll
+    for (int i = 0; i < HDP / 2; ++i) dq[i] = 0.f;
+
+    auto issue_sdp = [&]() {
+      const uint32_t kb = sK + ist * Cfg::KTILE, vb = sV + ist * Cfg::KTILE;
+#pragma unroll
+      for (int kk = 0; kk < HDP / 16; ++kk) {
+        const uint32_t qoff = (kk >> 2) * 16384 + (kk & 3) * 32, koff = (kk >> 2) * 8192 + (kk & 3) * 32;
+        WgmmaSS<64, 0, 0>::mma(s, make_smem_desc_sw128(qb + qoff, 0, 1024), make_smem_desc_sw128(kb + koff, 0, 1024),
+                               kk ? 1u : 0u);
+      }
+#pragma unroll
+      for (int kk = 0; kk < HDP / 16; ++kk) {
+        const uint32_t qoff = (kk >> 2) * 16384 + (kk & 3) * 32, koff = (kk >> 2) * 8192 + (kk & 3) * 32;
+        WgmmaSS<64, 0, 0>::mma(dp, make_smem_desc_sw128(dob + qoff, 0, 1024), make_smem_desc_sw128(vb + koff, 0, 1024),
+                               kk ? 1u : 0u);
+      }
+      wgmma_commit();
+      if (++ist == STAGES) { ist = 0; iph ^= 1u; }
+    };
+    auto issue_dq = [&]() {
+      const uint32_t kb = sK + rst * Cfg::KTILE;
+#pragma unroll
+      for (int kk = 0; kk < 4; ++kk)
+        WgmmaRS<HDP, 1>::mma(dq, da[kk], make_smem_desc_sw128(kb + kk * 2048, 8192, 1024), 1u);
+      wgmma_commit();
+    };
+    auto release_kv = [&]() {
+      if (wg_leader) mbar_arrive(kv_empty(rst));
+      if (++rst == STAGES) rst = 0;
+    };
+    auto tile_full = [&](int k0) {
+      bool full = k0 + 64 <= p.Skv && wq0 + 16 <= p.Sq && (!p.causal || k0 + 63 <= wq0 + coff);
+      if (full && km) full = keys_all_valid<64>(km, k0);
+      return full;
+    };
+    auto grads = [&](int k0, auto full_tile) {
 #pragma unroll
       for (int jj = 0; jj < 8; ++jj) {
-        float dsv[4];
 #pragma unroll
         for (int e = 0; e < 4; ++e) {
           const int r = e >> 1, key = k0 + 8 * jj + cq + (e & 1);
@@ -607,36 +741,71 @@
           if (!decltype(full_tile)::value)
             vis = qi[r] < p.Sq && key < p.Skv && (!p.causal || key <= qi[r] + coff) && (!km || km[key]);
           const float pe = vis ? fast_exp2(fmaf(s[4 * jj + e], p.scale_log2, -L[r])) : 0.f;
-          dsv[e] = pe * (dp[4 * jj + e] - D[r]);
+          s[4 * jj + e] = pe * (dp[4 * jj + e] - D[r]);
         }
-        da[jj >> 1][(jj & 1) * 2 + 0] = pack_bf16x2(dsv[0], dsv[1]);
-        da[jj >> 1][(jj & 1) * 2 + 1] = pack_bf16x2(dsv[2], dsv[3]);
-      }
-    };
-    if (full)
-      grads(std::true_type());
-    else
-      grads(std::false_type());
+      }
+    };
+    auto wait_grads = [&](int k0, bool full, auto wait) {
+      wait();
+      reg_fence(s);
+      reg_fence(dp);
+      if (full)
+        grads(k0, std::true_type());
+      else
+        grads(k0, std::false_type());
+    };
+    auto pack = [&]() {
+#pragma unroll
+      for (int jj = 0; jj < 8; ++jj) {
+        da[jj >> 1][(jj & 1) * 2 + 0] = pack_bf16x2(s[4 * jj + 0], s[4 * jj + 1]);
+        da[jj >> 1][(jj & 1) * 2 + 1] = pack_bf16x2(s[4 * jj + 2], s[4 * jj + 3]);
+      }
+    };
+
+    mbar_wait(q_full(qs), qph);
+    mbar_wait(kv_full(ist), iph);
+    named_bar_sync(bar_mine, 256);
+    wgmma_fence();
+    issue_sdp();
+    named_bar_arrive(bar_other, 256);
+    wait_grads(0, tile_full(0), [] { wgmma_wait<0>(); });
+    pack();
+    for (int j = 0; j + 1 < n_tiles; ++j) {
+      mbar_wait(kv_full(ist), iph);
+      named_bar_sync(bar_mine, 256);
+      reg_fence(dq);
+      wgmma_fence();
+      issue_sdp();
+      issue_dq();
+      named_bar_arrive(bar_other, 256);
+      const int k1 = (j + 1) * 64;
+      wait_grads(k1, tile_full(k1), [] { wgmma_wait<1>(); });
+      wgmma_wait<0>();
+      reg_fence(dq);
+      release_kv();
+      pack();
+    }
+    named_bar_sync(bar_mine, 256);
     reg_fence(dq);
     wgmma_fence();
-#pragma unroll
-    for (int kk = 0; kk < 4; ++kk)
-      WgmmaRS<HDP, 1>::mma(dq, da[kk], make_smem_desc_sw128(kb + kk * 2048, 8192, 1024), 1u);
-    wgmma_commit();
+    issue_dq();
+    named_bar_arrive(bar_other, 256);
     wgmma_wait<0>();
     reg_fence(dq);
-    if (wg_leader) mbar_arrive(kv_empty(st));
-    if (++st == STAGES) { st = 0; ph ^= 1u; }
-  }
-#pragma unroll
-  for (int r = 0; r < 2; ++r) {
-    if (qi[r] >= p.Sq) continue;
-    bf16* dqp = p.dq + (long long)b * p.dq_bs + (long long)qi[r] * p.dq_ss + (long long)h * p.hd;
-#pragma unroll
-    for (int jj = 0; jj < HDP / 8; ++jj)
-      *reinterpret_cast<__nv_bfloat162*>(dqp + 8 * jj + cq) =
-          __floats2bfloat162_rn(dq[4 * jj + 2 * r] * p.scale, dq[4 * jj + 2 * r + 1] * p.scale);
-  }
+    release_kv();
+    if (wg_leader) mbar_arrive(q_empty(qs));
+    if (++qs == 2) { qs = 0; qph ^= 1u; }
+#pragma unroll
+    for (int r = 0; r < 2; ++r) {
+      if (qi[r] >= p.Sq) continue;
+      bf16* dqp = p.dq + (long long)b * p.dq_bs + (long long)qi[r] * p.dq_ss + (long long)h * p.hd;
+#pragma unroll
+      for (int jj = 0; jj < HDP / 8; ++jj)
+        *reinterpret_cast<__nv_bfloat162*>(dqp + 8 * jj + cq) =
+            __floats2bfloat162_rn(dq[4 * jj + 2 * r] * p.scale, dq[4 * jj + 2 * r + 1] * p.scale);
+    }
+  }
+  if (wg == 0) named_bar_sync(1, 256);
 }
 
 static PFN_cuTensorMapEncodeTiled_v12000 encode_fn() {
@@ -677,8 +846,8 @@
 static int hd_padded(int hd) { return (hd + 15) / 16 * 16; }
 
 template <int HDP>
-static int launch_fwd(const CUtensorMap& tq, const CUtensorMap& tk, const CUtensorMap& tv, const AttnParams& p,
-                      cudaStream_t st) {
+static int launch_fwd(const CUtensorMap& tq, const CUtensorMap& tk, const CUtensorMap& tv, const CUtensorMap& to,
+                      const AttnParams& p, cudaStream_t st) {
   using Cfg = FwdCfg<HDP>;
   auto kern = attn_fwd_kernel<HDP>;
   static bool attr = false;
@@ -687,7 +856,8 @@
     if (e != cudaSuccess) return set_error(CB_ERR_CUDA, "attn fwd smem attr: %s", cudaGetErrorString(e));
     attr = true;
   }
-  kern<<<(p.Sq + 127) / 128 * p.nh * p.B, 288, Cfg::SMEM, st>>>(tq, tk, tv, p);
+  const long long work = (long long)(p.Sq + 127) / 128 * p.nh * p.B;
+  kern<<<(unsigned)std::min<long long>(work, device_sm_count()), 384, Cfg::SMEM, st>>>(tq, tk, tv, to, p);
   CB_CUDA_LAUNCH_CHECK("attn_fwd");
   return CB_OK;
 }
@@ -699,22 +869,25 @@
   CB_CHECK_ARG(B > 0 && nh > 0 && nkv > 0 && Sq > 0 && Skv > 0, "attention: empty problem");
   CB_CHECK_ARG(nh % nkv == 0, "attention: nh=%d not a multiple of nkv=%d", nh, nkv);
   CB_CHECK_ARG(hd % 8 == 0 && hd <= 128, "attention: head_dim=%d must be a multiple of 8 and <= 128", hd);
-  CB_CHECK_ARG(o_ss % 8 == 0 && o_bs % 8 == 0 && !(reinterpret_cast<uintptr_t>(o) & 15u),
-               "attention: output must be 16-byte aligned with strides %% 8 == 0");
-  CUtensorMap tq, tk, tv;
+  CB_CHECK_ARG(o_ss % 2 == 0 && o_bs % 2 == 0 && !(reinterpret_cast<uintptr_t>(o) & 3u),
+               "attention: output must be 4-byte aligned with even strides");
+  CUtensorMap tq, tk, tv, to;
   int rc;
   if ((rc = make_tmap_bf16_4d(&tq, q, hd, nh, Sq, B, hd, q_ss, q_bs, 128))) return rc;
   if ((rc = make_tmap_bf16_4d(&tk, k, hd, nkv, Skv, B, hd, k_ss, k_bs, 128))) return rc;
   if ((rc = make_tmap_bf16_4d(&tv, v, hd, nkv, Skv, B, hd, v_ss, v_bs, 128))) return rc;
+  const int tma_store = !(reinterpret_cast<uintptr_t>(o) & 15u) && o_ss % 8 == 0 && (B == 1 || o_bs % 8 == 0);
+  if (tma_store && (rc = make_tmap_bf16_4d(&to, o, hd, nh, Sq, B, hd, o_ss, o_bs, 64))) return rc;
   AttnParams p;
   p.o = (bf16*)o; p.o_bs = o_bs; p.o_ss = o_ss; p.lse = lse; p.kmask = (const uint8_t*)kmask;
   p.B = B; p.nh = nh; p.nkv = nkv; p.Sq = Sq; p.Skv = Skv; p.hd = hd; p.causal = causal;
   p.scale_log2 = scale * LOG2E;
+  p.tma_store = tma_store;
   const int hdp = hd_padded(hd);
-  if (hdp <= 64) return launch_fwd<64>(tq, tk, tv, p, st);
-  if (hdp <= 80) return launch_fwd<80>(tq, tk, tv, p, st);
-  if (hdp <= 96) return launch_fwd<96>(tq, tk, tv, p, st);
-  return launch_fwd<128>(tq, tk, tv, p, st);
+  if (hdp <= 64) return launch_fwd<64>(tq, tk, tv, to, p, st);
+  if (hdp <= 80) return launch_fwd<80>(tq, tk, tv, to, p, st);
+  if (hdp <= 96) return launch_fwd<96>(tq, tk, tv, to, p, st);
+  return launch_fwd<128>(tq, tk, tv, to, p, st);
 }
 
 template <int HDP>
@@ -744,7 +917,8 @@
     if (e != cudaSuccess) return set_error(CB_ERR_CUDA, "attn bwd dq smem attr: %s", cudaGetErrorString(e));
     attr = true;
   }
-  kern<<<(p.Sq + 127) / 128 * p.nh * p.B, 288, Cfg::SMEM, st>>>(tq, tk, tv, tdo, p);
+  const long long work = (long long)(p.Sq + 127) / 128 * p.nh * p.B;
+  kern<<<(unsigned)std::min<long long>(work, device_sm_count()), 384, Cfg::SMEM, st>>>(tq, tk, tv, tdo, p);
   CB_CUDA_LAUNCH_CHECK("attn_bwd_dq");
   return CB_OK;
 }
diff --git a/cambrian_b200/csrc/common.cuh b/cambrian_b200/csrc/common.cuh
--- a/cambrian_b200/csrc/common.cuh
+++ b/cambrian_b200/csrc/common.cuh
@@ -182,7 +182,13 @@
                : "l"(m), "r"(smem_src), "r"(c0), "r"(c1), "r"(c2)
                : "memory");
 }
-__device__ __forceinline__ void bulk_commit() { asm volatile("cp.async.bulk.commit_group;" ::: "memory"); }
+__device__ __forceinline__ void tma_store_4d(const CUtensorMap* m, uint32_t smem_src, int c0, int c1, int c2, int c3) {
+  asm volatile("cp.async.bulk.tensor.4d.global.shared::cta.bulk_group [%0, {%2, %3, %4, %5}], [%1];"
+               :
+               : "l"(m), "r"(smem_src), "r"(c0), "r"(c1), "r"(c2), "r"(c3)
+               : "memory");
+}
+__device__ __forceinline__ void bulk_commit(){ asm volatile("cp.async.bulk.commit_group;" ::: "memory"); }
 template <int N>
 __device__ __forceinline__ void bulk_wait_read() {
   asm volatile("cp.async.bulk.wait_group.read %0;" ::"n"(N) : "memory");
@@ -197,6 +203,9 @@
 __device__ __forceinline__ void setmaxnreg_inc() { asm volatile("setmaxnreg.inc.sync.aligned.u32 %0;" ::"n"(N)); }
 __device__ __forceinline__ void named_bar_sync(int id, int threads) {
   asm volatile("bar.sync %0, %1;" ::"r"(id), "r"(threads) : "memory");
+}
+__device__ __forceinline__ void named_bar_arrive(int id, int threads) {
+  asm volatile("bar.arrive %0, %1;" ::"r"(id), "r"(threads) : "memory");
 }
 
 __device__ __forceinline__ void wgmma_fence() { asm volatile("wgmma.fence.sync.aligned;" ::: "memory"); }
```

Result: no change. 7.956 (median of 6 runs) (+0.5%).
